# rsutormin/KmerGutsJava

Measured on AMD Instinct MI355X. Metric: amino-acid residues/sec scanned (and hits/sec) on 1 Gbp synthetic, 1/2/4/8 MI355X, higher is better.
Workload: dtype int64; 1 GPU; 1 Gbp contig mix (0.5 kbp..1.024 Mbp, uniform ACGT) on 1 GPU, 6-frame translate + 8-mer lookup vs 1400303159-slot signature table (33.6 GB, load 0.50), -m 5 -g 200; total_bp_rank0=1000000000, contigs_rank0=6351, total_bp_all_ranks=1000000000, num_sigs=1400303159, residues_rank0=1999974596, residues_all_ranks=1999974596, hits_rank0=36744843, hits_all_ranks=36744843, calls_rank0=4, parallelism=contig shards x1, table replicated

## Files before the change

kmergutsjava_amd/csrc/kg_host.hpp:

```cpp
#pragma once

#include <algorithm>
#include <atomic>
#include <cstdio>
#include <cstdlib>
#include <cstring>
#include <map>
#include <memory>
#include <mutex>
#include <new>
#include <optional>
#include <string>
#include <thread>
#include <unordered_map>
#include <vector>

namespace {

thread_local std::string g_err;

int fail(int code, const std::string &msg)
{
    g_err = msg;
    return code;
}

#define HIP_TRY(expr)                                                                              \
    do {                                                                                           \
        hipError_t e_ = (expr);                                                                    \
        if (e_ != hipSuccess)                                                                      \
            return fail(KG_ERR_DEVICE, std::string(#expr) + ": " + hipGetErrorString(e_));         \
    } while (0)

struct DevCache {
    std::mutex mu;
    std::multimap<size_t, void *> free_;
    std::unordered_map<void *, size_t> live;

    static size_t round_up(size_t b)
    {
        if (b < 256) return 256;
        size_t g = b >= (8u << 20) ? (2u << 20) : 256;
        return (b + g - 1) / g * g;
    }
    hipError_t get(void **p, size_t bytes)
    {
        bytes = round_up(bytes);
        std::lock_guard<std::mutex> lk(mu);
        auto it = free_.lower_bound(bytes);
        if (it != free_.end() && it->first <= bytes + bytes / 2 + (1u << 20)) {
            *p = it->second;
            live[*p] = it->first;
            free_.erase(it);
            return hipSuccess;
        }
        hipError_t e = hipMalloc(p, bytes);
        if (e != hipSuccess) {
            for (auto &kv : free_) (void)hipFree(kv.second);
            free_.clear();
            e = hipMalloc(p, bytes);
            if (e != hipSuccess) return e;
        }
        live[*p] = bytes;
        return hipSuccess;
    }
    void put(void *p)
    {
        std::lock_guard<std::mutex> lk(mu);
        auto it = live.find(p);
        if (it == live.end()) return;
        free_.emplace(it->second, p);
        live.erase(it);
    }
    void detach(void *p)
    {
        std::lock_guard<std::mutex> lk(mu);
        live.erase(p);
    }
    size_t live_bytes()
    {
        std::lock_guard<std::mutex> lk(mu);
        size_t n = 0;
        for (auto &kv : live) n += kv.second;
        return n;
    }
    void release_all()
    {
        std::lock_guard<std::mutex> lk(mu);
        for (auto &kv : free_) (void)hipFree(kv.second);
        for (auto &kv : live) (void)hipFree(kv.first);
        free_.clear();
        live.clear();
    }
    void release_free()
    {
        std::lock_guard<std::mutex> lk(mu);
        for (auto &kv : free_) (void)hipFree(kv.second);
        free_.clear();
    }
};

struct PinCache {
    std::mutex mu;
    std::multimap<size_t, void *> free_;
    std::unordered_map<void *, size_t> live;
    size_t kept = 0;
    static constexpr size_t kKeepTotal = 6ull << 30;

    hipError_t get(void **p, size_t bytes)
    {
        bytes = bytes < 4096 ? 4096 : (bytes + 4095) / 4096 * 4096;
        {
            std::lock_guard<std::mutex> lk(mu);
            auto it = free_.lower_bound(bytes);
            if (it != free_.end() && it->first <= 2 * bytes + (1u << 16)) {
                *p = it->second;
                live[*p] = it->first;
                kept -= it->first;
                free_.erase(it);
                return hipSuccess;
            }
        }
        hipError_t e = hipHostMalloc(p, bytes);
        if (e != hipSuccess) return e;
        std::lock_guard<std::mutex> lk(mu);
        live[*p] = bytes;
        return hipSuccess;
    }
    void put(void *p)
    {
        std::vector<void *> drop;
        {
            std::lock_guard<std::mutex> lk(mu);
            auto it = live.find(p);
            if (it == live.end()) return;
            const size_t bytes = it->second;
            live.erase(it);
            free_.emplace(bytes, p);
            kept += bytes;
            while (kept > kKeepTotal && !free_.empty()) {
                auto big = std::prev(free_.end());
                kept -= big->first;
                drop.push_back(big->second);
                free_.erase(big);
            }
        }
        for (void *d : drop) (void)hipHostFree(d);
    }
    void release_all()
    {
        std::lock_guard<std::mutex> lk(mu);
        for (auto &kv : free_) (void)hipHostFree(kv.second);
        for (auto &kv : live) (void)hipHostFree(kv.first);
        free_.clear();
        live.clear();
        kept = 0;
    }
};

}

constexpr uint64_t kHbitsMaxSlots = 1ull << 26;

constexpr uint32_t kMaxChunks = 8;
constexpr uint32_t kMaxOrderStreams = 4;
enum : int {
    kPevChunk = 0,
    kPevFork = 16,
    kPevJoin2 = 17, kPevJoin3 = 18,
    kPevTotals = 19,
    kPevVerified = 20,
    kPevBase = 32,
    kPevOrdered = 40,
    kPevCount = 48
};
static_assert(kPevChunk + 2 * kMaxChunks <= kPevFork && kPevVerified + kMaxChunks <= kPevBase && kPevBase + kMaxChunks <= kPevOrdered &&
              kPevOrdered + kMaxOrderStreams <= kPevCount, "event slots overlap");
enum : int { kEvBegin = 0, kEvScanBegin = 1, kEvScanEnd = 2, kEvOrderEnd = 3, kEvAggEnd = 4, kEvScattered = 5 , kEvSpare = 6,
             kEvJoined = 7 , kEvCount = 8, kEvStageBegin = kEvBegin, kEvStageEnd = kEvScanBegin };
enum : int { kTotHits = 0, kTotCursor = 1 , kTotValid = 2, kTotSlots = 3 ,
             kTotCalls = 4, kTotRanOff = 5 , kTotPieces = 6, kTotVoters = 7, kTotWords = 8,
             kTotSent = 6  };
enum : int { kPcUcur = 0 , kPcCcur = 8 , kPcBase = 16 ,
             kPcCtot = 32 , kPcWords = 48 };
static_assert(kPcUcur + kMaxChunks <= kPcCcur && kPcCcur + kMaxChunks <= kPcBase && kPcBase + kMaxChunks + 1 <= kPcCtot &&
              kPcCtot + kMaxChunks <= kPcWords, "per-chunk words overlap");
enum : int { kOvfGroups = 0 , kOvfLowc = 1 , kOvfGuard = 2 ,
             kOvfWords = 8 };
enum : int { kPinPc = 0 , kPinOvf = 48 , kPinTotals = 80 , kPinCalls = 88 ,
             kPinPieces = 89, kPinWords = 96,
             kPinStage = 80, kPinStageWords = kPinWords - kPinStage,
             kPinAssign = 90  };
static_assert(kPinPc + kPcWords <= kPinOvf && kOvfWords * kMaxChunks * 4 <= (kPinTotals - kPinOvf) * 8 && kPinTotals + kTotSent <= kPinCalls,
              "counters must fit their pinned words");
static_assert(kPinAssign >= kPinStage && kPinAssign + 2 + 3 <= kPinWords, "stage words must fit their pinned words");

struct kg_table {
    int device = 0;
    hipStream_t stream = nullptr;
    hipStream_t stream2 = nullptr;
    hipStream_t stream3 = nullptr;
    hipStream_t ostream[kMaxOrderStreams] = {};
    hipEvent_t pev[kPevCount] = {};
    bool own_entries = false;
    uint8_t *d_entries = nullptr;
    uint8_t *d_tags = nullptr;
    uint8_t *d_bidx = nullptr;
    bool bidx_exact = false;
    uint32_t *d_hbits = nullptr;
    uint64_t tail_start = 0;
    int64_t num_sigs = 0, entry_size = 0, version = 0;
    uint64_t limit = 0;
    uint64_t magic = 0;
    uint32_t m35 = 0;
    uint64_t occupied = 0;
    double stage_ratio = 1.0 / 16;
    size_t scatter_lds[2][3] = {};
    kg::ScatterCold *d_cold = nullptr;
    kg::ScatterCold h_cold[kMaxChunks] = {};
    kg::CallsCold *d_calls_cold = nullptr;
    kg::CallsCold h_calls_cold = {};
    size_t hist_lds = 48 * 1024;
    size_t place_lds[2] = {48 * 1024, 48 * 1024};
    hipEvent_t ev[kEvCount] = {};
    uint64_t *h_pin = nullptr;
    std::atomic<int> busy{0};
    uint32_t fail_alloc_at = 0, alloc_count = 0;
    DevCache cache;
    PinCache pins;
};

struct kg_result {
    kg_table *tab = nullptr;
    bool own_tab = false;
    kg_stats st = {};
    uint32_t per = 6;
    kg_hit *d_hits = nullptr;
    int64_t *d_chs = nullptr;
    kg_call *d_calls = nullptr;
    int64_t *d_ccs = nullptr;
    kg_otu *d_otu = nullptr;
    uint8_t *d_ev = nullptr, *d_tail_ev = nullptr;
    uint32_t *d_hit_slots = nullptr;
    bool has_progress = false;
    kg_progress progress = {};
    void *h_hits = nullptr, *h_chs = nullptr, *h_ccs = nullptr, *h_calls = nullptr, *h_otu = nullptr, *h_ev = nullptr,
         *h_tail_ev = nullptr, *h_hit_slots = nullptr;
};

namespace {

uint32_t env_u32(const char *name, uint32_t dflt)
{
    const char *v = getenv(name);
    if (!v || !*v) return dflt;
    char *end = nullptr;
    long x = strtol(v, &end, 10);
    return (end != v && x >= 0) ? (uint32_t)x : dflt;
}

constexpr uint32_t kMaxGrid = 256u * 32u;

uint32_t env_knob(const char *name, uint32_t dflt, uint32_t lo, uint32_t hi, uint32_t mult = 1)
{
    uint32_t x = dflt;
    if (const char *v = getenv(name); v && *v) {
        char *end = nullptr;
        const long long y = strtoll(v, &end, 10);
        if (end != v && y >= 0) x = y > (long long)hi ? hi : (uint32_t)y;
    }
    x = std::min(hi, std::max(lo, x));
    return (x + mult - 1) / mult * mult;
}

uint32_t test_hook(const char *name)
{
    static const bool enabled = env_u32("KG_ENABLE_TEST_HOOKS", 0u) != 0;
    return enabled ? env_u32(name, 0u) : 0u;
}

int dalloc(kg_table *t, void **p, size_t bytes)
{
    if (t->fail_alloc_at && ++t->alloc_count == t->fail_alloc_at)
        return fail(KG_ERR_NOMEM, "device allocation failed: KG_TEST_FAIL_ALLOC test hook");
    hipError_t e = t->cache.get(p, bytes);
    if (e != hipSuccess) return fail(KG_ERR_NOMEM, std::string("device allocation failed: ") + hipGetErrorString(e));
    return KG_OK;
}

void dfree(kg_table *t, void *p)
{
    if (p) t->cache.put(p);
}

int dalloc_detached(kg_table *t, uint8_t **p, size_t bytes)
{
    const int rc = dalloc(t, (void **)p, bytes);
    if (rc == KG_OK) t->cache.detach(*p);
    return rc;
}

struct Detached {
    uint8_t *p = nullptr;
    Detached() = default;
    Detached(const Detached &) = delete;
    Detached &operator=(const Detached &) = delete;
    ~Detached() { if (p) (void)hipFree(p); }
};

int table_new(int device, kg_table **out);

struct CallScope {
    kg_table *t = nullptr;
    const bool owned;
    int rc;
    CallScope(kg_table *tab, const char *busy_text) : owned(false), rc(tab->busy.exchange(1) != 0 ? fail(KG_ERR_BUSY, busy_text) : KG_OK)
    {
        if (rc == KG_OK) { t = tab; rc = arm(true); }
    }
    explicit CallScope(int device, bool hook = true) : owned(true), rc(table_new(device, &t))
    {
        if (rc == KG_OK) arm(hook);
    }
    ~CallScope()
    {
        if (!t) return;
        t->fail_alloc_at = 0;
        if (owned) kg_table_close(t);
        else t->busy.store(0);
    }
    int arm(bool hook)
    {
        t->fail_alloc_at = hook ? test_hook("KG_TEST_FAIL_ALLOC") : 0u;
        t->alloc_count = 0;
        if (!owned) HIP_TRY(hipSetDevice(t->device));
        return KG_OK;
    }
    kg_table *disown() { kg_table *out = t; t = nullptr; out->fail_alloc_at = 0; return out; }
};

int prefix_sum(kg_table *t, const uint32_t *d_in, uint64_t n, uint32_t *d_out, uint64_t *d_partial, uint64_t *d_total,
               hipStream_t stream = nullptr)
{
    if (!stream) stream = t->stream;
    uint32_t nb = (uint32_t)((n + kg::kScanChunk - 1) / kg::kScanChunk);
    if (nb == 0) nb = 1;
    hipLaunchKernelGGL(kg::scan_partials_kernel, dim3(nb), dim3(kg::kScanThreads), 0, stream, d_in, n, d_partial);
    hipLaunchKernelGGL(kg::scan_top_kernel, dim3(1), dim3(kg::kScanThreads), 0, stream, d_partial, nb, d_total);
    hipLaunchKernelGGL(kg::scan_final_kernel, dim3(nb), dim3(kg::kScanThreads), 0, stream, d_in, n, d_partial, d_out);
    HIP_TRY(hipGetLastError());
    return KG_OK;
}

struct ClearItem { void *p; uint64_t words; };

template <typename G>
int clear_words(hipStream_t stream, G grid, std::initializer_list<ClearItem> items)
{
    kg::ClearList cl = {};
    uint64_t most = 0;
    for (const ClearItem &it : items) {
        if (!it.words) continue;
        if (cl.n == (int)std::size(cl.p)) return fail(KG_ERR_DEVICE, "more than eight arrays in one clear (internal error)");
        cl.p[cl.n] = (uint32_t *)it.p; cl.words[cl.n++] = it.words;
        most = std::max(most, it.words);
    }
    if (cl.n) hipLaunchKernelGGL(kg::clear_many_kernel, dim3(grid(most)), dim3(256), 0, stream, cl);
    return KG_OK;
}

struct Scratch {
    kg_table *t;
    std::vector<void *> ptrs;
    explicit Scratch(kg_table *tt) : t(tt) {}
    ~Scratch()
    {
        (void)hipStreamSynchronize(t->stream);
        if (t->stream2) (void)hipStreamSynchronize(t->stream2);
        if (t->stream3) (void)hipStreamSynchronize(t->stream3);
        for (auto &os : t->ostream) if (os) (void)hipStreamSynchronize(os);
        for (void *p : ptrs) dfree(t, p);
    }
    void adopt(void *p) { ptrs.push_back(p); }
    void release(void *p) { ptrs.erase(std::find(ptrs.begin(), ptrs.end(), p)); }
    template <typename T> int get(T **p, size_t count)
    {
        void *v = nullptr;
        int rc = dalloc(t, &v, count * sizeof(T));
        if (rc) return rc;
        ptrs.push_back(v);
        *p = (T *)v;
        return KG_OK;
    }
};

struct SetBase {
    kg_table *tab = nullptr;
    bool own_tab = false;
    std::vector<void *> blocks;
    SetBase() = default;
    SetBase(const SetBase &) = delete;
    SetBase &operator=(const SetBase &) = delete;
    ~SetBase()
    {
        if (!tab) return;
        (void)hipSetDevice(tab->device);
        for (void *p : blocks) dfree(tab, p);
        if (own_tab) kg_table_close(tab);
    }
    template <typename T> T *keep(Scratch &sc, T *p)
    {
        if (p) { blocks.push_back(p); sc.release(p); }
        return p;
    }
};

template <typename S>
int make_set(const CallScope &cs, std::unique_ptr<S> &set)
{
    set.reset(new (std::nothrow) S());
    if (!set) return fail(KG_ERR_NOMEM, "out of host memory");
    set->tab = cs.t;
    return KG_OK;
}

template <typename S>
int hand_out(CallScope &cs, std::unique_ptr<S> &set, S **out)
{
    if (cs.owned) {
        cs.t->cache.release_free();
        set->own_tab = true;
        cs.disown();
    }
    *out = set.release();
    return KG_OK;
}

int device_of(const SetBase *s) { return s ? s->tab->device : 0; }

template <typename T>
int copy_records(const void *s, int device, const T *src, size_t per, int64_t have, int64_t first, int64_t count, T *dst, const char *what,
                 const char *of = "the set")
{
    if (!s || (count > 0 && !dst)) return fail(KG_ERR_ARG, "null argument");
    if (first < 0 || count < 0 || first + count > have) return fail(KG_ERR_ARG, std::string(what) + ": range outside " + of);
    if (count == 0) return KG_OK;
    HIP_TRY(hipSetDevice(device));
    HIP_TRY(hipMemcpy(dst, src + (size_t)first * per, (size_t)count * per * sizeof(T), hipMemcpyDefault));
    return KG_OK;
}

int copy_starts(const void *s, int device, const int64_t *src, int64_t n, int64_t *dst)
{
    if (!s || !dst) return fail(KG_ERR_ARG, "null argument");
    HIP_TRY(hipSetDevice(device));
    HIP_TRY(hipMemcpy(dst, src, ((size_t)n + 1) * 8, hipMemcpyDefault));
    return KG_OK;
}

template <typename St>
int copy_stats(const void *s, const St *st, St *out)
{
    if (!s || !out) return fail(KG_ERR_ARG, "null argument");
    *out = *st;
    return KG_OK;
}

uint32_t grid_of(uint64_t n, uint32_t threads = 256)
{
    return (uint32_t)std::max<uint64_t>(1, (n + threads - 1) / threads);
}

uint64_t magic_of(uint64_t d)
{
    return d == 1 ? ~0ull : (uint64_t)(((unsigned __int128)1 << 64) / d);
}

std::string kmer_text(int64_t v)
{
    char b[32];
    snprintf(b, sizeof b, "%lld", (long long)v);
    return b;
}

int fail_and_free(kg_result *r, int rc) { std::string keep = g_err; kg_result_free(r); g_err = keep; return rc; }

uint32_t bit_width(uint64_t v) { return v ? 64u - (uint32_t)__builtin_clzll(v) : 0u; }

uint32_t bits_for(uint64_t n) { return n > 1 ? bit_width(n - 1) : 0; }

template <int N>
struct Events {
    hipEvent_t e[N] = {};
    ~Events() { for (auto x : e) if (x) (void)hipEventDestroy(x); }
    int create() { for (auto &x : e) HIP_TRY(hipEventCreate(&x)); return KG_OK; }
    hipEvent_t operator[](int i) const { return e[i]; }
    float ms(int i, int j) const { float m = 0; (void)hipEventElapsedTime(&m, e[i], e[j]); return m; }
};

struct ErrWord { int word, code; const char *prefix, *suffix; };
constexpr uint64_t kNoErr = 0x7F7F7F7F7F7F7F7Full;
static_assert(kNoErr == kg::kAssignNoErr && kNoErr == kg::kRegionNoErr, "the stages' kernels share the error words' \"none\"");

int read_error_words(kg_table *t, const void *d_words, size_t n_words, int pin, std::initializer_list<ErrWord> table)
{
    HIP_TRY(hipMemcpyAsync(t->h_pin + pin, d_words, n_words * 8, hipMemcpyDeviceToHost, t->stream));
    HIP_TRY(hipStreamSynchronize(t->stream));
    for (const ErrWord &w : table)
        if (const uint64_t at = t->h_pin[pin + w.word]; at != kNoErr) return fail(w.code, w.prefix + kmer_text((int64_t)at) + w.suffix);
    return KG_OK;
}

int read_record_errors(kg_table *t, const void *d_words, size_t n_words, int n_err, const char *const *what)
{
    int rc;
    if ((rc = read_error_words(t, d_words, n_words, kPinStage, {}))) return rc;
    const uint64_t *h = t->h_pin + kPinStage;
    const int first = (int)(std::min_element(h, h + n_err) - h);
    if (h[first] != kNoErr) return fail(KG_ERR_ARG, "record " + kmer_text((int64_t)h[first]) + what[first]);
    return KG_OK;
}

int upload_pinned(kg_table *t, const uint8_t *src, size_t bytes, uint8_t *d_dst)
{
    const size_t CH = 32u << 20;
    const size_t n_pieces = (bytes + CH - 1) / CH;
    const unsigned hw = std::thread::hardware_concurrency();
    const size_t n_thr = std::max<size_t>(1, std::min<size_t>({(size_t)8, (size_t)(hw ? hw : 4), n_pieces}));
    std::atomic<size_t> next{0};
    std::atomic<bool> ok{true};
    auto worker = [&]() {
        if (hipSetDevice(t->device) != hipSuccess) { ok = false; return; }
        hipStream_t s = nullptr;
        uint8_t *pin[2] = {nullptr, nullptr};
        hipEvent_t done[2] = {nullptr, nullptr};
        bool good = hipStreamCreateWithFlags(&s, hipStreamNonBlocking) == hipSuccess &&
                    hipHostMalloc((void **)&pin[0], CH) == hipSuccess && hipHostMalloc((void **)&pin[1], CH) == hipSuccess &&
                    hipEventCreate(&done[0]) == hipSuccess && hipEventCreate(&done[1]) == hipSuccess;
        bool used[2] = {false, false};
        int which = 0;
        while (good && ok.load()) {
            const size_t k = next.fetch_add(1);
            if (k >= n_pieces) break;
            const size_t at = k * CH, n = std::min(CH, bytes - at);
            if (used[which]) good = hipEventSynchronize(done[which]) == hipSuccess;
            if (!good) break;
            memcpy(pin[which], src + at, n);
            good = hipMemcpyAsync(d_dst + at, pin[which], n, hipMemcpyHostToDevice, s) == hipSuccess &&
                   hipEventRecord(done[which], s) == hipSuccess;
            used[which] = true;
            which ^= 1;
        }
        if (s && hipStreamSynchronize(s) != hipSuccess) good = false;
        if (!good) ok = false;
        for (int i = 0; i < 2; i++) { if (pin[i]) (void)hipHostFree(pin[i]); if (done[i]) (void)hipEventDestroy(done[i]); }
        if (s) (void)hipStreamDestroy(s);
    };
    {
        std::vector<std::thread> pool;
        for (size_t i = 1; i < n_thr; i++) pool.emplace_back(worker);
        worker();
        for (auto &th : pool) th.join();
    }
    return ok.load() ? KG_OK : fail(KG_ERR_DEVICE, "uploading to the device failed (pinned staging or host-to-device copy)");
}

struct SortPairs {
    uint64_t *k[2] = {nullptr, nullptr};
    uint32_t *v[2] = {nullptr, nullptr};
    int cur = 0;
    int alloc(Scratch &sc, uint64_t n) { int rc = sc.get(&k[0], n); return rc ? rc : sc.get(&v[0], n); }
    uint64_t *keys() const { return k[cur]; }
    uint32_t *vals() const { return v[cur]; }
    SortPairs next() const { SortPairs s; s.k[0] = k[cur ^ 1]; s.v[0] = v[cur]; return s; }
    int sort(kg_table *t, Scratch &sc, uint64_t n, uint32_t key_bits);
};

int SortPairs::sort(kg_table *t, Scratch &sc, uint64_t n, uint32_t key_bits)
{
    if (n <= 1 || key_bits == 0) return KG_OK;
    const uint32_t n_tiles = (uint32_t)((n + kg::kBuildTile - 1) / kg::kBuildTile);
    const uint32_t passes = (key_bits + 7) / 8, bits = passes ? (key_bits + passes - 1) / passes : 1, radix = 1u << bits;
    const uint64_t n_hist = (uint64_t)radix * n_tiles;
    const uint64_t nb = (n_hist + kg::kScanChunk - 1) / kg::kScanChunk;
    uint32_t *hist = nullptr, *offs = nullptr;
    uint64_t *partial = nullptr;
    int rc;
    if ((rc = sc.get(&k[cur ^ 1], n)) || (rc = sc.get(&v[cur ^ 1], n)) || (rc = sc.get(&hist, n_hist)) ||
        (rc = sc.get(&offs, n_hist)) || (rc = sc.get(&partial, nb + 2)))
        return rc;
    for (uint32_t p = 0; p < passes; p++) {
        const uint32_t shift = p * bits;
        hipLaunchKernelGGL(kg::build_hist_kernel, dim3(n_tiles), dim3(kg::kBuildThreads), 0, t->stream, k[cur], n, shift, radix,
                           n_tiles, hist);
        HIP_TRY(hipGetLastError());
        if ((rc = prefix_sum(t, hist, n_hist, offs, partial, partial + nb + 1))) return rc;
        hipLaunchKernelGGL(kg::build_scatter_kernel, dim3(n_tiles), dim3(kg::kBuildThreads), 0, t->stream, k[cur], v[cur], n,
                           shift, bits, n_tiles, offs, k[cur ^ 1], v[cur ^ 1]);
        HIP_TRY(hipGetLastError());
        cur ^= 1;
    }
    return KG_OK;
}

}
```

kmergutsjava_amd/csrc/kg_host_plan.hpp:

```cpp
#pragma once

namespace {


template <typename T, T V, T... Vs, typename F>
void dispatch(T x, F &&f)
{
    if constexpr (sizeof...(Vs) == 0) f(std::integral_constant<T, V>{});
    else if (x == V) f(std::integral_constant<T, V>{});
    else dispatch<T, Vs...>(x, f);
}

struct BatchPlan {
    std::vector<uint32_t> ibase;
    uint64_t nblocks = 0, windows = 0, residues = 0;
    uint64_t n_rows = 0, n_cont = 0;
    int64_t longest = 0;
};

template <bool AA>
int plan_batch(const int64_t *offsets, int64_t n_seqs, BatchPlan &b)
{
    constexpr uint32_t PER = AA ? 1 : 6;
    b.ibase.resize((size_t)n_seqs + 1);
    for (int64_t k = 0; k < n_seqs; k++) {
        int64_t L = offsets[k + 1] - offsets[k];
        if (L < 0) return fail(KG_ERR_ARG, "offsets must be non-decreasing");
        b.longest = std::max(b.longest, L);
        if (L > 0xFFFFFFF0ll) return fail(KG_ERR_LIMIT, "a single sequence longer than 2^32-16 characters");
        b.ibase[(size_t)k] = (uint32_t)b.nblocks;
        uint64_t nb;
        if (AA) {
            uint64_t nwin = L >= 9 ? (uint64_t)L - 8 : 0;
            b.windows += nwin;
            b.residues += (uint64_t)L;
            nb = (nwin + kg::kAaWinPerBlock - 1) / kg::kAaWinPerBlock;
        } else {
            uint64_t npos = L >= 24 ? (uint64_t)L - 23 : 0;
            b.windows += 2 * npos;
            for (int f = 0; f < 3; f++)
                if (L - f >= 3) b.residues += 2 * (uint64_t)((L - f) / 3);
            nb = (npos + kg::kDnaPosPerBlock - 1) / kg::kDnaPosPerBlock;
        }
        b.nblocks += nb;
        if (b.nblocks > 0x7FFFFFFFull / PER) return fail(KG_ERR_LIMIT, "batch too large: more than 2^31-1 window rows; split the batch");
    }
    b.ibase[(size_t)n_seqs] = (uint32_t)b.nblocks;
    if (b.windows > 0xFFFFFF00ull) return fail(KG_ERR_LIMIT, "batch too large: more than 2^32-256 windows; split the batch");
    b.n_rows = b.nblocks * PER;
    b.n_cont = (uint64_t)n_seqs * PER;
    return KG_OK;
}

uint64_t bucket_count(uint64_t limit, uint32_t shift) { return (limit + (1ull << shift) - 1) >> shift; }

struct PartPlan {
    bool applicable = false;
    uint32_t shift = 0, buckets = 0;
    uint32_t n_chunks = 0;
    std::vector<uint64_t> clo;
    std::vector<int64_t> cseq;
    uint64_t max_chunk = 0;
    uint32_t n_wg = 0, cap = 0;
    uint64_t n_regions = 0;
    uint32_t ovf_cap = 0;
    uint32_t gshift = 10, groups_stride = 0;
    size_t next_stride = 0;
    size_t scatter_lds = 0;
    bool use_bidx = false, part_counters = false, prog_index = false;
    uint32_t probe_grid = 0, index_grid = 0, verify_grid = 0, lowc_grid = 0, ovf_grid = 0, order_grid = 0;
    uint32_t scatter_prio = 0, index_prio = 0, verify_prio = 0, index_r = 1, probe_grab = 0;
    uint32_t flush_list = 0;
    uint64_t list_slack = 0, ucap = 0, ccap = 0;
    uint32_t n_os = 0;
    bool early_totals = false, place_staged = false, debug = false;
};

template <bool AA>
int plan_partition(const kg_table *t, const BatchPlan &b, bool progress, bool counters_req, PartPlan &pl)
{
    constexpr uint32_t PER = AA ? 1 : 6;
    const uint64_t nblocks = b.nblocks;
    uint32_t shift = env_knob("KG_PART_SHIFT", 21u, 4u, 31u);
    const uint64_t qmax = (uint64_t)KG_MAX_ENCODED / (uint64_t)t->num_sigs + 1;
    while (shift > 4 && qmax >= (1ull << (32 - shift))) shift--;
    while (bucket_count(t->limit, shift) > (uint64_t)kg::kMaxBuckets) shift++;
    while (kg::scatter_lds_bytes<AA>((uint32_t)bucket_count(t->limit, shift)) > 160u * 1024) shift++;
    const bool fits = shift < 32 && qmax < (1ull << (32 - shift)) && nblocks <= (1ull << 23) && t->m35 != 0 &&
                      t->limit < (1ull << 32) - 64;
    const uint32_t mode = env_u32("KG_PARTITION", 2u);
    const bool worth = t->limit >= (64ull << 20) && b.windows >= (1ull << 27);
    if (!(fits && nblocks > 0 && (mode == 1 || (mode == 2 && worth)))) return KG_OK;
    pl.shift = shift;
    pl.buckets = (uint32_t)bucket_count(t->limit, shift);

    constexpr uint32_t WIN = AA ? 64u : 384u;
    uint32_t want = env_u32("KG_PART_CHUNKS", 4u);
    if (want < 1) want = 1;
    if (want > kMaxChunks) want = kMaxChunks;
    if (getenv("KG_PART_MIN_CHUNK_BLOCKS")) {
        const uint64_t min_chunk = std::max(1u, env_u32("KG_PART_MIN_CHUNK_BLOCKS", 600000u));
        while (want > 1 && nblocks / want < min_chunk) want--;
    } else {
        const uint32_t by_size = nblocks < 450000 ? 1u : std::max(2u, (uint32_t)std::lround(std::sqrt((double)nblocks / 325000.0)));
        want = std::min(want, std::max(1u, by_size));
    }
    pl.clo.push_back(0); pl.cseq.push_back(0);
    std::vector<double> cum;
    if (const char *tp = getenv("KG_PART_TAPER")) {
        double acc = 0;
        for (const char *q = tp; *q;) {
            char *endp = nullptr;
            const double v = strtod(q, &endp);
            if (endp == q) break;
            acc += v; cum.push_back(acc);
            q = *endp == ',' ? endp + 1 : endp;
        }
        if (cum.size() >= 2 && cum.size() <= kMaxChunks && acc > 0) { for (auto &x : cum) x /= acc; want = (uint32_t)cum.size(); }
        else cum.clear();
    }
    for (uint32_t c = 1; c < want; c++) {
        const uint64_t target = cum.empty() ? nblocks * c / want : (uint64_t)((double)nblocks * cum[c - 1]);
        const auto it = std::lower_bound(b.ibase.begin(), b.ibase.end(), (uint32_t)target);
        const uint64_t cut = *it;
        if (cut > pl.clo.back() && cut < nblocks) { pl.clo.push_back(cut); pl.cseq.push_back((int64_t)(it - b.ibase.begin())); }
    }
    pl.clo.push_back(nblocks); pl.cseq.push_back((int64_t)b.ibase.size() - 1);
    pl.n_chunks = (uint32_t)pl.clo.size() - 1;
    for (uint32_t c = 0; c < pl.n_chunks; c++) pl.max_chunk = std::max(pl.max_chunk, pl.clo[c + 1] - pl.clo[c]);
    const uint64_t max_chunk = pl.max_chunk;
    const uint64_t chunk_blocks = (max_chunk + kg::kScatterWaves - 1) / kg::kScatterWaves * kg::kScatterWaves;
    const double max_frac = (double)max_chunk / (double)nblocks;
    uint32_t n_wg = env_knob("KG_PART_WGS", 256u, 1u, kMaxGrid);
    if ((uint64_t)n_wg * kg::kScatterWaves > chunk_blocks) n_wg = (uint32_t)((chunk_blocks + kg::kScatterWaves - 1) / kg::kScatterWaves);
    const uint64_t blocks_per_wg = ((chunk_blocks + (uint64_t)n_wg * kg::kScatterWaves - 1) / ((uint64_t)n_wg * kg::kScatterWaves)) * kg::kScatterWaves;
    const double mean = (double)blocks_per_wg * WIN / (double)pl.buckets * (env_u32("KG_PART_SLACK", 100u) / 100.0);
    const uint64_t cap64 = ((uint64_t)(mean + 6.0 * std::sqrt(mean) + 32.0) + 15) / 16 * 16;
    if (cap64 >= (1ull << 24) || (uint64_t)pl.buckets * n_wg >= (1ull << 24)) return KG_OK;
    pl.n_wg = n_wg;
    pl.cap = (uint32_t)cap64;
    pl.n_regions = (uint64_t)pl.buckets * n_wg;
    pl.ovf_cap = env_u32("KG_PART_OVF_GROUPS", (uint32_t)std::min<uint64_t>(1u << 23, std::max<uint64_t>(65536, pl.n_regions * pl.cap / 16 / 8)));
    while (pl.gshift < 12 && ((max_chunk * PER) >> pl.gshift) + 2 > 8192) pl.gshift++;
    pl.groups_stride = (uint32_t)(((max_chunk * PER) >> pl.gshift) + 2);
    if (pl.groups_stride > kg::kMaxGroups) return fail(KG_ERR_LIMIT, "a chunk of the batch holds more than 2^26 window rows");
    pl.next_stride = std::max<size_t>((size_t)pl.buckets + 8, 256);
    pl.use_bidx = t->d_bidx != nullptr && !counters_req && env_u32("KG_BIDX", 1u) != 0;
    pl.part_counters = (counters_req || progress) && !pl.use_bidx;
    pl.prog_index = progress && pl.use_bidx;
    pl.scatter_lds = kg::scatter_lds_bytes<AA>(pl.buckets);
    pl.flush_list = env_knob("KG_SCATTER_FLUSH_LIST", kg::scatter_flush_list_max<AA>(), 1u, kg::scatter_flush_list_max<AA>());
    pl.probe_grid = env_knob("KG_PROBE_GRID", 256u * 8u, 8u, kMaxGrid, 8u);
    pl.index_grid = env_knob("KG_INDEX_GRID", 256u * 4u, 8u, kMaxGrid, 8u);
    pl.scatter_prio = std::min(3u, env_u32("KG_SCATTER_PRIO", 1u));
    pl.index_prio = std::min(3u, env_u32("KG_INDEX_PRIO", 2u));
    pl.verify_prio = std::min(3u, env_u32("KG_VERIFY_PRIO", pl.n_chunks == 1 ? 2u : 0u));
    uint32_t index_r = env_u32("KG_INDEX_R", 0u);
    if (index_r == 0) index_r = mean * 0.7 >= 640.0 ? 1u : mean * 0.7 >= 320.0 ? 2u : 4u;
    if (index_r != 1 && index_r != 2) index_r = 4;
    while (index_r > 1 && (n_wg % index_r != 0 || kg::kIndexN % index_r != 0)) index_r /= 2;
    pl.index_r = index_r;
    pl.verify_grid = env_knob("KG_VERIFY_GRID", 256u * 2u, 1u, kMaxGrid);
    pl.lowc_grid = env_knob("KG_LOWC_GRID", 256u, 1u, kMaxGrid);
    pl.ovf_grid = env_knob("KG_OVF_GRID", 256u, 1u, kMaxGrid);
    pl.list_slack = (uint64_t)(std::max(std::max(pl.probe_grid, pl.index_grid), pl.verify_grid) + 64) * 4 * kg::kUChunk + 4096;
    pl.ucap = ((uint64_t)((double)b.windows * t->stage_ratio * max_frac) + pl.list_slack + kg::kUChunk - 1) / kg::kUChunk * kg::kUChunk;
    pl.ccap = ((uint64_t)((double)b.windows * (t->stage_ratio * 1.25 + 0.03) * max_frac) + pl.list_slack + kg::kUChunk - 1) /
              kg::kUChunk * kg::kUChunk;
    if (test_hook("KG_TEST_TINY_LISTS")) pl.ucap = pl.ccap = kg::kUChunk;
    const uint32_t grab_unit = 256u * (uint32_t)std::max(kg::kProbeN, kg::kIndexN);
    pl.probe_grab = env_knob("KG_PROBE_GRAB", pl.cap, grab_unit, 1u << 24, grab_unit);
    pl.n_os = pl.n_chunks < 2 ? 0u : std::min(env_u32("KG_ORDER_STREAMS", 0u), kMaxOrderStreams);
    pl.early_totals = pl.n_os == 0 && env_u32("KG_EARLY_TOTALS", 1u) != 0;
    pl.order_grid = env_knob("KG_ORDER_GRID", 256u * 3u, 1u, kMaxGrid);
    pl.place_staged = pl.gshift == 10 && env_u32("KG_PLACE_STAGED", 1u) != 0;
    pl.debug = getenv("KG_DEBUG") != nullptr;
    pl.applicable = true;
    return KG_OK;
}

struct DirectPlan {
    uint32_t scan_grid, stage_chunk;
    const uint32_t *d_hbits;
    uint32_t rpg;
    uint64_t stage_cap;
};

template <bool AA>
DirectPlan plan_direct(const kg_table *t, const BatchPlan &b, bool counters)
{
    DirectPlan pl;
    pl.scan_grid = env_knob("KG_SCAN_GRID", 256u * 8u, 1u, kMaxGrid);
    pl.stage_chunk = env_knob("KG_STAGE_CHUNK", 256u, 1u, 1u << 12);
    const uint32_t filter_mode = env_u32("KG_DIRECT_FILTER", 1u);
    pl.d_hbits = (counters || filter_mode == 0 || (filter_mode == 1 && t->limit <= (4ull << 20))) ? nullptr : t->d_hbits;
    pl.rpg = AA ? 1u : env_u32("KG_SCAN_RPG", pl.d_hbits ? 6u : 3u);
    if (pl.rpg != 1 && pl.rpg != 2 && pl.rpg != 3 && pl.rpg != 6) pl.rpg = 3;
    pl.stage_cap = (uint64_t)((double)b.windows * t->stage_ratio) + 4096 + (uint64_t)pl.scan_grid * kg::kWavesPerWG * pl.stage_chunk;
    if (pl.stage_cap > 0xFFFFFF00ull) pl.stage_cap = 0xFFFFFF00ull;
    if (test_hook("KG_TEST_TINY_LISTS")) pl.stage_cap = 256;
    return pl;
}

struct AggPlan {
    uint32_t pshift;
    bool pieces_on;
    uint32_t agg_pairs;
};

AggPlan plan_aggregate()
{
    AggPlan pl;
    pl.pshift = std::min(20u, std::max(6u, env_u32("KG_AGG_BLOCK_SHIFT", 9u)));
    pl.pieces_on = env_u32("KG_AGG_PIECES", 1u) != 0;
    pl.agg_pairs = env_u32("KG_AGG_PAIRS", 1u);
    return pl;
}

}
```

kmergutsjava_amd/csrc/kg_host_scan.hpp:

```cpp
#pragma once

namespace {

struct ScanCtx {
    kg_table *t;
    kg_result *res;
    Scratch &sc;
    const BatchPlan &b;
    const uint8_t *d_seq, *h_seq;
    const int64_t *offsets;
    int64_t n_seqs;
    bool progress, counters;
    bool seq_uploaded;
    uint64_t n_hits = 0;
    int64_t *d_off = nullptr;
    uint32_t *d_ibase = nullptr;
    kg::BlockDesc *d_blocks = nullptr;
    uint32_t *d_counts = nullptr, *d_offs = nullptr, *d_bsb = nullptr;
    uint64_t *d_partial = nullptr, *d_totals = nullptr;
    kg::Progress *d_prog = nullptr;
};

int upload_seq(const ScanCtx &cx, int64_t a, int64_t b)
{
    if (cx.h_seq && b > a)
        HIP_TRY(hipMemcpyAsync(const_cast<uint8_t *>(cx.d_seq) + a, cx.h_seq + a, (size_t)(b - a), hipMemcpyHostToDevice, cx.t->stream));
    return KG_OK;
}

template <int N>
struct BlockGuard {
    Scratch &sc;
    void **slot[N];
    void release() { for (void **q : slot) { dfree(sc.t, *q); *q = nullptr; } }
    ~BlockGuard() { for (void **q : slot) if (*q) { sc.adopt(*q); *q = nullptr; } }
};

void drop_hits(kg_table *t, kg_result *res)
{
    dfree(t, res->d_hits); dfree(t, res->d_hit_slots);
    res->d_hits = nullptr; res->d_hit_slots = nullptr;
}

int send_counters(kg_table *t, const uint64_t *d_pc, const uint32_t *d_ovfc, const uint64_t *d_totals, hipStream_t s)
{
    if (d_pc) {
        HIP_TRY(hipMemcpyAsync(t->h_pin + kPinPc, d_pc, kPcWords * 8, hipMemcpyDeviceToHost, s));
        HIP_TRY(hipMemcpyAsync(t->h_pin + kPinOvf, d_ovfc, kOvfWords * kMaxChunks * 4, hipMemcpyDeviceToHost, s));
    }
    HIP_TRY(hipMemcpyAsync(t->h_pin + kPinTotals, d_totals, kTotSent * 8, hipMemcpyDeviceToHost, s));
    return KG_OK;
}

void note_totals(ScanCtx &cx, uint64_t n_hits, bool counted)
{
    kg_table *t = cx.t;
    kg_stats &st = cx.res->st;
    const uint64_t *h_tot = t->h_pin + kPinTotals;
    st.windows_valid = counted ? (int64_t)h_tot[kTotValid] : -1;
    st.slots_inspected = counted ? (int64_t)h_tot[kTotSlots] : -1;
    st.lookup_ran_off = h_tot[kTotRanOff] ? 1 : 0;
    if (cx.b.windows) {
        double ratio = (double)n_hits / (double)cx.b.windows * 1.1 + 1e-3;
        if (ratio > t->stage_ratio) t->stage_ratio = ratio > 1.0 ? 1.0 : ratio;
    }
    cx.n_hits = n_hits;
    st.n_hits = (int64_t)n_hits;
}

int progress_begin(ScanCtx &cx)
{
    kg_table *t = cx.t;
    int rc;
    if (t->limit > 0xFFFFFFFFull) return fail(KG_ERR_UNSUPPORTED, "KG_F_PROGRESS: table streams of 2^32 records or more");
    if ((rc = cx.sc.get(&cx.d_prog, 1))) return rc;
    kg::Progress h;
    for (auto &x : h.first) x = ~0ull;
    h.last_plus1 = 0; h.first_beyond = ~0ull; h.walk_ran_off = 0;
    for (auto &x : h.found_upto) x = 0;
    h.kmers_found = 0;
    for (auto &x : h.miss_max1) x = 0;
    const double n = (double)t->num_sigs;
    auto tenth = [&](uint64_t s) { return (int)(10.0 * ((double)(s + 1) / n)); };
    for (int f = 0; f <= 10; f++) {
        const unsigned __int128 num = (unsigned __int128)(uint64_t)t->num_sigs * (unsigned)f;
        uint64_t s = (uint64_t)((num + 9) / 10);
        s = s > 3 ? s - 3 : 0;
        while (tenth(s) < f) s++;
        h.lo[f] = s;
    }
    HIP_TRY(hipMemcpyAsync(cx.d_prog, &h, sizeof h, hipMemcpyHostToDevice, t->stream));
    HIP_TRY(hipStreamSynchronize(t->stream));
    return KG_OK;
}

int progress_finish(ScanCtx &cx, bool index_walks)
{
    kg_table *t = cx.t;
    int rc;
    if (index_walks)
        hipLaunchKernelGGL(kg::progress_finish_kernel, dim3(1), dim3(256), 0, t->stream, cx.d_prog, t->d_tags, t->limit);
    uint32_t *d_bitmap = nullptr;
    const uint64_t n_words = (t->limit + 31) / 32 + 1;
    if ((rc = cx.sc.get(&d_bitmap, (size_t)n_words))) return rc;
    HIP_TRY(hipMemsetAsync(d_bitmap, 0, n_words * 4, t->stream));
    if (cx.n_hits)
        hipLaunchKernelGGL(kg::mark_found_kernel, dim3((uint32_t)std::min<uint64_t>(2048, (cx.n_hits + 255) / 256)), dim3(256), 0, t->stream,
                           cx.res->d_hit_slots, cx.n_hits, d_bitmap);
    hipLaunchKernelGGL(kg::count_found_kernel, dim3((uint32_t)std::min<uint64_t>(2048, (n_words + 255) / 256)), dim3(256), 0, t->stream,
                       d_bitmap, n_words, cx.d_prog);
    return KG_OK;
}

int progress_fetch(ScanCtx &cx)
{
    kg::Progress h;
    HIP_TRY(hipMemcpy(&h, cx.d_prog, sizeof h, hipMemcpyDeviceToHost));
    kg_progress &g = cx.res->progress;
    for (int f = 0; f <= 10; f++) g.first_visited[f] = h.first[f] == ~0ull ? -1 : (int64_t)h.first[f];
    g.last_visited = (int64_t)h.last_plus1 - 1;
    g.first_beyond = h.first_beyond == ~0ull ? -1 : (int64_t)h.first_beyond;
    g.walk_ran_off = h.walk_ran_off ? 1 : 0;
    g.stream_slots = (int64_t)cx.t->limit;
    for (int f = 0; f <= 10; f++) g.found_upto[f] = g.first_visited[f] < 0 ? 0 : (int64_t)h.found_upto[f];
    g.kmers_found = (int64_t)h.kmers_found;
    cx.res->has_progress = true;
    return KG_OK;
}

struct PartBuffers {
    uint64_t *d_ent = nullptr, *d_ovf_ent = nullptr;
    uint32_t *d_fill = nullptr, *d_ovf_bucket = nullptr, *d_next = nullptr;
    uint32_t *d_ovfc = nullptr;
    uint32_t *d_lowc = nullptr;
    kg::RowGeo *d_geo = nullptr;
    uint64_t *d_pc = nullptr;
    uint32_t *d_ghist = nullptr, *d_gbase = nullptr, *d_gcur1 = nullptr, *d_gcur2 = nullptr, *d_gtile = nullptr;
    uint64_t ucap = 0, ccap = 0;
    size_t cused_stride = 0, candused_stride = 0;
    kg_hit *d_ulist = nullptr, *d_sortA = nullptr, *d_sortB = nullptr;
    uint32_t *d_cused = nullptr, *d_candused = nullptr;
    kg::CandRec *d_cand = nullptr;
};

struct ChunkView {
    uint32_t c, lo, nb;
    uint64_t *ent, *ovf_ent;
    uint32_t *fill, *next, *ovfc, *ovf_bucket;
    kg_hit *ulist, *sortA, *sortB;
    uint32_t *cused, *candused;
    kg::CandRec *cand;
    unsigned long long *ucur, *ccur;
    uint64_t *base, *ctot;
    uint32_t *ghist, *gbase, *gcur1, *gcur2, *gtile;
};

ChunkView chunk_view(const PartPlan &pl, const PartBuffers &pb, uint32_t c)
{
    ChunkView v;
    v.c = c; v.lo = (uint32_t)pl.clo[c]; v.nb = (uint32_t)(pl.clo[c + 1] - pl.clo[c]);
    v.ent = pb.d_ent + (uint64_t)c * pl.n_regions * pl.cap;
    v.fill = pb.d_fill + (uint64_t)c * pl.n_regions;
    v.next = pb.d_next + (size_t)c * pl.next_stride;
    v.ovfc = pb.d_ovfc + kOvfWords * c; v.ovf_bucket = pb.d_ovf_bucket + (size_t)c * pl.ovf_cap;
    v.ovf_ent = pb.d_ovf_ent + (size_t)c * pl.ovf_cap * kg::kGroup;
    v.ulist = pb.d_ulist + (uint64_t)c * pb.ucap;
    v.cused = pb.d_cused + c * pb.cused_stride; v.candused = pb.d_candused + c * pb.candused_stride;
    v.cand = pb.d_cand + (uint64_t)c * pb.ccap;
    v.ucur = (unsigned long long *)(pb.d_pc + kPcUcur + c); v.ccur = (unsigned long long *)(pb.d_pc + kPcCcur + c);
    v.base = pb.d_pc + kPcBase + c; v.ctot = pb.d_pc + kPcCtot + c;
    v.ghist = pb.d_ghist + (size_t)c * pl.groups_stride; v.gbase = pb.d_gbase + (size_t)c * (pl.groups_stride + 1);
    v.gcur1 = pb.d_gcur1 + (size_t)c * (kg::kHDigits + 1); v.gcur2 = pb.d_gcur2 + (size_t)c * pl.groups_stride;
    v.gtile = pb.d_gtile + (size_t)c * (kg::kHDigits + 1);
    v.sortA = pb.d_sortA + (uint64_t)c * pb.ucap; v.sortB = pb.d_sortB + (uint64_t)c * pb.ucap;
    return v;
}

int scatter_variant_of(const ScanCtx &cx)
{
    return cx.t->limit >= (uint64_t)cx.t->num_sigs ? 0 : cx.d_prog ? 2 : 1;
}
template <typename F>
void scatter_variant(int variant, F &&f)
{
    if (variant == 0) f(std::false_type{}, std::false_type{});
    else if (variant == 1) f(std::true_type{}, std::false_type{});
    else f(std::true_type{}, std::true_type{});
}

int upload_scatter_cold(const ScanCtx &cx, const PartPlan &pl, const PartBuffers &pb)
{
    kg_table *t = cx.t;
    kg::ScatterCold h[kMaxChunks] = {};
    for (uint32_t c = 0; c < pl.n_chunks; c++) {
        uint32_t *ovfc = pb.d_ovfc + kOvfWords * c;
        h[c].ovf_cursor = ovfc; h[c].ovf_bucket = pb.d_ovf_bucket + (size_t)c * pl.ovf_cap;
        h[c].ovf_ent = pb.d_ovf_ent + (size_t)c * pl.ovf_cap * kg::kGroup;
        h[c].lowc_cursor = ovfc + kOvfLowc; h[c].lowc_blocks = pb.d_lowc + pl.clo[c];
        h[c].ctr = (unsigned long long *)(cx.d_totals + kTotValid); h[c].prog = cx.d_prog;
        h[c].ovf_cap = pl.ovf_cap;
    }
    if (!t->d_cold) HIP_TRY(hipMalloc((void **)&t->d_cold, sizeof h));
    else if (!memcmp(h, t->h_cold, sizeof h)) return KG_OK;
    memcpy(t->h_cold, h, sizeof h);
    HIP_TRY(hipMemcpyAsync(t->d_cold, t->h_cold, sizeof h, hipMemcpyHostToDevice, t->stream));
    return KG_OK;
}

template <bool AA>
int chunk_passes(const ScanCtx &cx, const PartPlan &pl, const PartBuffers &pb, const ChunkView &v)
{
    kg_table *t = cx.t;
    kg::Progress *d_prog = cx.d_prog;
    unsigned long long *d_ctr = (unsigned long long *)(cx.d_totals + kTotValid);
    const hipStream_t s2 = t->stream2, s3 = t->stream3;
    uint32_t *lowc_cursor = v.ovfc + kOvfLowc, *lowc = pb.d_lowc + v.lo;
    const uint32_t limit32 = (uint32_t)std::min<uint64_t>(t->limit, 0xFFFFFFFFull);
    scatter_variant(scatter_variant_of(cx), [&](auto is_short, auto prog) {
        constexpr bool SHORT = decltype(is_short)::value, PROG = decltype(prog)::value;
        hipLaunchKernelGGL((kg::part_scatter_kernel<AA, SHORT, PROG>), dim3(pl.n_wg), dim3(kg::kWave * kg::kScatterWaves), pl.scatter_lds,
                           t->stream, cx.d_seq, cx.d_blocks, v.lo, v.nb, limit32, (uint32_t)t->num_sigs, t->m35, pl.shift, pl.buckets, pl.cap,
                           v.ent, v.fill, t->d_cold + v.c, pl.scatter_prio, pl.flush_list);
    });
    HIP_TRY(hipEventRecord(t->pev[kPevChunk + 2 * v.c], t->stream));
    HIP_TRY(hipStreamWaitEvent(s2, t->pev[kPevChunk + 2 * v.c], 0));
    hipLaunchKernelGGL((kg::lowc_blocks_kernel<AA>), dim3(pl.lowc_grid), dim3(64 * kg::kLowcWaves), 0, s2, cx.d_seq, cx.d_blocks, lowc_cursor, lowc,
                       t->limit, (uint32_t)t->num_sigs, t->m35, pl.shift, pl.n_wg, pl.cap, v.ent, v.fill, v.ovfc, pl.ovf_cap,
                       v.ovf_bucket, v.ovf_ent, d_ctr, d_prog);
    if (pl.use_bidx) {
        const uint32_t tail_start = (uint32_t)std::min<uint64_t>(t->tail_start, 0xFFFFFFFFull);
        dispatch<int, 1, 2, 4>((int)pl.index_r, [&](auto r) {
            dispatch<bool, true, false>(t->bidx_exact, [&](auto exact) {
                dispatch<bool, true, false>(pl.prog_index, [&](auto prog) {
                    constexpr int R = decltype(r)::value;
                    constexpr bool EXACT = decltype(exact)::value, PROG = decltype(prog)::value;
                    hipLaunchKernelGGL((kg::bucket_index_kernel<kg::kIndexN, R, EXACT, PROG>), dim3(pl.index_grid), dim3(256), 0, s2,
                                       t->d_bidx, tail_start, v.ent, v.fill, pl.n_wg, pl.cap, pl.buckets, pl.shift, pl.probe_grab, v.next,
                                       v.cand, v.candused, v.ccur, pb.ccap, d_ctr, pl.index_prio, PROG ? d_prog : (kg::Progress *)nullptr);
                });
            });
        });
    } else {
        dispatch<bool, true, false>(pl.part_counters, [&](auto counters) {
            constexpr bool COUNTERS = decltype(counters)::value;
            hipLaunchKernelGGL((kg::bucket_tag_kernel<COUNTERS>), dim3(pl.probe_grid), dim3(256), 0, s2, t->d_tags, t->limit,
                               (uint64_t)t->num_sigs, v.ent, v.fill, pl.n_wg, pl.cap, pl.buckets, pl.shift, pl.probe_grab, v.next, v.cand,
                               v.candused, v.ccur, pb.ccap, d_ctr, COUNTERS ? d_prog : (kg::Progress *)nullptr);
        });
    }
    HIP_TRY(hipEventRecord(t->pev[kPevChunk + 2 * v.c + 1], s2));
    HIP_TRY(hipStreamWaitEvent(s3, t->pev[kPevChunk + 2 * v.c + 1], 0));
    dispatch<int, 1, 2, 0>(pl.part_counters ? 1 : pl.prog_index ? 2 : 0, [&](auto walks) {
        constexpr bool COUNTERS = decltype(walks)::value == 1, PROG = decltype(walks)::value == 2;
        hipLaunchKernelGGL((kg::verify_kernel<AA, COUNTERS, PROG>), dim3(pl.verify_grid), dim3(256), 0, s3, t->d_entries, t->d_tags, t->limit,
                           (uint64_t)t->num_sigs, t->magic, v.cand, v.candused, v.ccur, pb.ccap, v.ulist, v.cused, v.ucur, pb.ucap, d_ctr,
                           d_prog, pl.verify_prio);
        hipLaunchKernelGGL((kg::overflow_probe_kernel<AA, COUNTERS, PROG>), dim3(pl.ovf_grid), dim3(256), 0, s3, t->d_entries, t->d_tags,
                           t->limit, (uint64_t)t->num_sigs, t->magic, v.ovf_bucket, v.ovf_ent, v.ovfc, pl.ovf_cap, pl.shift, v.ulist,
                           v.cused, v.ucur, pb.ucap, d_ctr, d_prog);
    });
    HIP_TRY(hipEventRecord(t->pev[kPevVerified + v.c], s3));
    HIP_TRY(hipGetLastError());
    return KG_OK;
}

template <bool AA>
int chunk_order(const ScanCtx &cx, const PartPlan &pl, const PartBuffers &pb, const ChunkView &v, uint64_t hits_cap)
{
    constexpr uint32_t PER = AA ? 1 : 6;
    kg_table *t = cx.t;
    kg_result *res = cx.res;
    const uint32_t c = v.c, gshift = pl.gshift;
    const bool last = c + 1 == pl.n_chunks;
    hipStream_t s = t->stream;
    if (pl.n_os) {
        s = t->ostream[c % pl.n_os];
        HIP_TRY(hipStreamWaitEvent(s, t->ev[kEvScattered], 0));
    }
    HIP_TRY(hipStreamWaitEvent(s, t->pev[kPevVerified + c], 0));
    const uint64_t row_lo = (uint64_t)v.lo * PER, row_hi = row_lo + (uint64_t)v.nb * PER;
    const uint32_t g0 = (uint32_t)(row_lo >> gshift);
    const uint32_t n_groups = v.nb ? (uint32_t)(((row_hi - 1) >> gshift) - g0 + 1) : 1u;
    hipLaunchKernelGGL(kg::hit_hist_kernel, dim3(pl.order_grid), dim3(kg::kHThreads), (size_t)n_groups * 4, s, v.ulist, v.cused, v.ucur, pb.ucap,
                       g0, 6u + gshift, n_groups, v.ghist);
    hipLaunchKernelGGL(kg::group_scan_kernel, dim3(1), dim3(kg::kGsThreads), 0, s, v.ghist, n_groups, v.gbase, v.gcur1, v.gcur2, v.ctot, v.gtile);
    if (pl.n_os && c) HIP_TRY(hipStreamWaitEvent(s, t->pev[kPevBase + c - 1], 0));
    hipLaunchKernelGGL(kg::chunk_base_kernel, dim3(1), dim3(1), 0, s, v.ctot, v.base, last ? cx.d_totals : (uint64_t *)nullptr);
    if (pl.n_os) HIP_TRY(hipEventRecord(t->pev[kPevBase + c], s));
    if (pl.early_totals && last) {
        int rc;
        if ((rc = send_counters(t, pb.d_pc, pb.d_ovfc, cx.d_totals, s))) return rc;
        HIP_TRY(hipEventRecord(t->pev[kPevTotals], s));
    }
    hipLaunchKernelGGL((kg::hit_partition_kernel<true>), dim3(pl.order_grid), dim3(kg::kHThreads), 0, s, v.ulist, v.cused, v.ucur, pb.ucap,
                       v.gbase, n_groups, g0, 6u + gshift, v.gcur1, v.sortA, pb.ucap, v.gtile);
    hipLaunchKernelGGL((kg::hit_partition_kernel<false>), dim3(pl.order_grid), dim3(kg::kHThreads), 0, s, v.sortA, v.cused, v.ucur, pb.ucap,
                       v.gbase, n_groups, g0, 6u + gshift, v.gcur2, v.sortB, pb.ucap, v.gtile);
    hipLaunchKernelGGL((kg::group_place_kernel<AA>), dim3(std::min(n_groups, 256u * 8u)), dim3(kg::kHThreads),
                       kg::group_place_lds(gshift, pl.place_staged), s,
                       v.sortB, v.gbase, n_groups, g0, gshift, (uint32_t)row_lo, (uint32_t)row_hi, pb.d_geo, (uint64_t)cx.b.n_rows,
                       pl.place_staged ? 1u : 0u, v.base, res->d_hits, hits_cap, cx.d_offs, res->d_hit_slots);
    HIP_TRY(hipGetLastError());
    return KG_OK;
}

template <bool AA>
int part_allocate(ScanCtx &cx, const PartPlan &pl, PartBuffers &pb)
{
    kg_table *t = cx.t;
    Scratch &sc = cx.sc;
    const uint32_t n_chunks = pl.n_chunks, groups_stride = pl.groups_stride;
    int rc;
    if ((rc = sc.get(&pb.d_ent, (size_t)(pl.n_regions * pl.cap * n_chunks)))) return rc;
    if ((rc = sc.get(&pb.d_fill, (size_t)pl.n_regions * n_chunks))) return rc;
    if ((rc = sc.get(&pb.d_ovf_ent, (size_t)pl.ovf_cap * kg::kGroup * n_chunks))) return rc;
    if ((rc = sc.get(&pb.d_ovf_bucket, (size_t)pl.ovf_cap * n_chunks))) return rc;
    if ((rc = sc.get(&pb.d_next, pl.next_stride * n_chunks))) return rc;
    if ((rc = sc.get(&pb.d_ovfc, kOvfWords * kMaxChunks))) return rc;
    if ((rc = sc.get(&pb.d_lowc, (size_t)cx.b.nblocks + 1))) return rc;
    if ((rc = sc.get(&pb.d_geo, (size_t)cx.b.n_rows))) return rc;
    if ((rc = sc.get(&pb.d_ghist, (size_t)groups_stride * n_chunks))) return rc;
    if ((rc = sc.get(&pb.d_gbase, (size_t)(groups_stride + 1) * n_chunks))) return rc;
    if ((rc = sc.get(&pb.d_gcur1, (size_t)(kg::kHDigits + 1) * n_chunks))) return rc;
    if ((rc = sc.get(&pb.d_gcur2, (size_t)groups_stride * n_chunks))) return rc;
    if ((rc = sc.get(&pb.d_gtile, (size_t)(kg::kHDigits + 1) * n_chunks))) return rc;
    if (kg::group_place_lds(pl.gshift, pl.gshift == 10) > t->place_lds[AA ? 1 : 0]) {
        const size_t want_lds = kg::group_place_lds(pl.gshift, pl.gshift == 10);
        HIP_TRY(hipFuncSetAttribute((const void *)kg::group_place_kernel<AA>, hipFuncAttributeMaxDynamicSharedMemorySize, (int)want_lds));
        t->place_lds[AA ? 1 : 0] = want_lds;
    }
    if (groups_stride * 4u > t->hist_lds) {
        HIP_TRY(hipFuncSetAttribute((const void *)kg::hit_hist_kernel, hipFuncAttributeMaxDynamicSharedMemorySize, (int)(groups_stride * 4u)));
        t->hist_lds = groups_stride * 4u;
    }
    if ((rc = sc.get(&pb.d_pc, kPcWords))) return rc;
    const int sv = scatter_variant_of(cx);
    if (t->scatter_lds[AA ? 1 : 0][sv] < pl.scatter_lds) {
        hipError_t e = hipSuccess;
        scatter_variant(sv, [&](auto is_short, auto prog) {
            e = hipFuncSetAttribute((const void *)kg::part_scatter_kernel<AA, decltype(is_short)::value, decltype(prog)::value>,
                                    hipFuncAttributeMaxDynamicSharedMemorySize, (int)pl.scatter_lds);
        });
        HIP_TRY(e);
        t->scatter_lds[AA ? 1 : 0][sv] = pl.scatter_lds;
    }
    return KG_OK;
}

template <bool AA>
int scan_partitioned(ScanCtx &cx, const PartPlan &pl, bool &done)
{
    constexpr uint32_t PER = AA ? 1 : 6;
    kg_table *t = cx.t;
    kg_result *res = cx.res;
    kg_stats &st = res->st;
    const uint32_t n_chunks = pl.n_chunks;
    const uint64_t nblocks = cx.b.nblocks;
    int rc;
    PartBuffers pb;
    if ((rc = part_allocate<AA>(cx, pl, pb))) return rc;
    BlockGuard<6> lists{cx.sc, {(void **)&pb.d_ulist, (void **)&pb.d_cused, (void **)&pb.d_cand, (void **)&pb.d_candused,
                                (void **)&pb.d_sortA, (void **)&pb.d_sortB}};
    pb.ucap = pl.ucap; pb.ccap = pl.ccap;
    HIP_TRY(hipEventRecord(t->ev[kEvScanBegin], t->stream));
    for (int attempt = 0; attempt < 3; attempt++) {
        const uint64_t ucap = pb.ucap, ccap = pb.ccap;
        const uint64_t hits_cap = ucap * n_chunks;
        pb.cused_stride = (size_t)(ucap / kg::kUChunk + 1); pb.candused_stride = (size_t)(ccap / kg::kUChunk + 1);
        if ((rc = dalloc(t, (void **)&res->d_hits, hits_cap * sizeof(kg_hit)))) return rc;
        if (cx.progress && (rc = dalloc(t, (void **)&res->d_hit_slots, hits_cap * 4))) return rc;
        if ((rc = dalloc(t, (void **)&pb.d_ulist, ucap * n_chunks * sizeof(kg_hit)))) return rc;
        if ((rc = dalloc(t, (void **)&pb.d_cused, pb.cused_stride * n_chunks * 4))) return rc;
        if ((rc = dalloc(t, (void **)&pb.d_cand, ccap * n_chunks * sizeof(kg::CandRec)))) return rc;
        if ((rc = dalloc(t, (void **)&pb.d_candused, pb.candused_stride * n_chunks * 4))) return rc;
        if ((rc = dalloc(t, (void **)&pb.d_sortA, ucap * n_chunks * sizeof(kg_hit)))) return rc;
        if ((rc = dalloc(t, (void **)&pb.d_sortB, ucap * n_chunks * sizeof(kg_hit)))) return rc;
        if ((rc = clear_words(t->stream, [](uint64_t most) { return (uint32_t)std::min<uint64_t>(4096, (most / 4 + 255) / 256 + 1); },
                              {{pb.d_cused, (uint64_t)pb.cused_stride * n_chunks},
                               {pb.d_candused, (uint64_t)pb.candused_stride * n_chunks},
                               {pb.d_pc, kPcWords * 2},
                               {cx.d_totals, kTotWords * 2},
                               {pb.d_ovfc, kOvfWords * kMaxChunks},
                               {pb.d_next, (uint64_t)pl.next_stride * n_chunks},
                               {pb.d_ghist, (uint64_t)pl.groups_stride * n_chunks}})))
            return rc;
        if ((rc = upload_scatter_cold(cx, pl, pb))) return rc;
        HIP_TRY(hipEventRecord(t->pev[kPevFork], t->stream));
        HIP_TRY(hipStreamWaitEvent(t->stream2, t->pev[kPevFork], 0));
        HIP_TRY(hipStreamWaitEvent(t->stream3, t->pev[kPevFork], 0));
        hipLaunchKernelGGL((kg::row_geo_kernel<AA>), dim3((uint32_t)((nblocks * PER + 255) / 256)), dim3(256), 0, t->stream3, cx.d_blocks,
                           (uint32_t)nblocks, pb.d_geo);
        for (uint32_t c = 0; c < n_chunks; c++) {
            if (!cx.seq_uploaded && (rc = upload_seq(cx, cx.offsets[pl.cseq[c]], cx.offsets[pl.cseq[c + 1]]))) return rc;
            if ((rc = chunk_passes<AA>(cx, pl, pb, chunk_view(pl, pb, c)))) return rc;
        }
        HIP_TRY(hipEventRecord(t->ev[kEvScattered], t->stream));
        cx.seq_uploaded = true;
        for (uint32_t k = 0; k < pl.n_os; k++)
            if (!t->ostream[k]) {
                int pr_least = 0, pr_greatest = 0;
                HIP_TRY(hipDeviceGetStreamPriorityRange(&pr_least, &pr_greatest));
                HIP_TRY(hipStreamCreateWithPriority(&t->ostream[k], hipStreamNonBlocking, pr_least));
            }
        for (uint32_t c = 0; c < n_chunks; c++)
            if ((rc = chunk_order<AA>(cx, pl, pb, chunk_view(pl, pb, c), hits_cap))) return rc;

        for (uint32_t k = 0; k < pl.n_os; k++) {
            HIP_TRY(hipEventRecord(t->pev[kPevOrdered + k], t->ostream[k]));
            HIP_TRY(hipStreamWaitEvent(t->stream, t->pev[kPevOrdered + k], 0));
        }
        HIP_TRY(hipEventRecord(t->pev[kPevJoin2], t->stream2));
        HIP_TRY(hipStreamWaitEvent(t->stream, t->pev[kPevJoin2], 0));
        HIP_TRY(hipEventRecord(t->pev[kPevJoin3], t->stream3));
        HIP_TRY(hipStreamWaitEvent(t->stream, t->pev[kPevJoin3], 0));
        HIP_TRY(hipEventRecord(t->ev[kEvJoined], t->stream));
        st.scan_launches++;
        HIP_TRY(hipEventRecord(t->ev[kEvScanEnd], t->stream));
        if (pl.early_totals) {
            HIP_TRY(hipEventSynchronize(t->pev[kPevTotals]));
        } else {
            if ((rc = send_counters(t, pb.d_pc, pb.d_ovfc, cx.d_totals, t->stream))) return rc;
            HIP_TRY(hipStreamSynchronize(t->stream));
        }
        const uint64_t *h_pc = t->h_pin + kPinPc;
        const uint32_t *h_ovf = reinterpret_cast<const uint32_t *>(t->h_pin + kPinOvf);
        uint64_t need_u = 0, need_c = 0;
        uint32_t max_ovf = 0, guard = 0;
        for (uint32_t c = 0; c < n_chunks; c++) {
            need_u = std::max(need_u, h_pc[kPcUcur + c]); need_c = std::max(need_c, h_pc[kPcCcur + c]);
            max_ovf = std::max(max_ovf, h_ovf[kOvfWords * c + kOvfGroups]);
            guard |= h_ovf[kOvfWords * c + kOvfGuard];
        }
        const uint64_t n_hits = h_pc[kPcBase + n_chunks];
        if (pl.debug)
            fprintf(stderr, "[kg] partition attempt %d: %u chunks (largest %llu of %llu blocks), overflow groups <= %u (cap %u), hit list <= %llu "
                            "(cap %llu), candidates <= %llu (cap %llu), regions/chunk %llu x %u entries, %u buckets, shift %u, %u scatter "
                            "workgroups, hits %llu, %s\n",
                    attempt, n_chunks, (unsigned long long)pl.max_chunk, (unsigned long long)nblocks, max_ovf, pl.ovf_cap,
                    (unsigned long long)need_u, (unsigned long long)ucap, (unsigned long long)need_c, (unsigned long long)ccap,
                    (unsigned long long)pl.n_regions, pl.cap, pl.buckets, pl.shift, pl.n_wg, (unsigned long long)n_hits, pl.use_bidx ? "byte home index" : "tags");
        const bool redo = guard || max_ovf > pl.ovf_cap || need_u > ucap || need_c > ccap;
        if (redo && pl.early_totals) HIP_TRY(hipStreamSynchronize(t->stream));
        if (guard || max_ovf > pl.ovf_cap) {
            st.fallback = guard ? 2 : 1;
            lists.release();
            drop_hits(t, res);
            return KG_OK;
        }
        if (!redo) {
            note_totals(cx, n_hits, pl.part_counters);
            st.partitioned = 1;
            st.part_chunks = (int32_t)n_chunks; st.part_buckets = (int32_t)pl.buckets; st.part_shift = (int32_t)pl.shift;
            st.part_levels = pl.use_bidx ? 4 : 1;
            done = true;
            return KG_OK;
        }
        lists.release();
        drop_hits(t, res);
        if (attempt == 2) break;
        if (need_c > ccap) { pb.ccap = (need_c + pl.list_slack + kg::kUChunk - 1) / kg::kUChunk * kg::kUChunk; pb.ucap = std::max(ucap, pb.ccap); }
        else pb.ucap = (need_u + pl.list_slack + kg::kUChunk - 1) / kg::kUChunk * kg::kUChunk;
    }
    return fail(KG_ERR_DEVICE, "hit list overflow after resize (internal error)");
}

template <bool AA>
int scan_direct(ScanCtx &cx, const DirectPlan &pl)
{
    kg_table *t = cx.t;
    kg_result *res = cx.res;
    kg_stats &st = res->st;
    const uint64_t nblocks = cx.b.nblocks, n_rows = cx.b.n_rows;
    int rc;
    st.scan_launches = 0;
    if (!cx.seq_uploaded) { if ((rc = upload_seq(cx, cx.offsets[0], cx.offsets[cx.n_seqs]))) return rc; cx.seq_uploaded = true; }
    uint64_t stage_cap = pl.stage_cap;
    kg_hit *d_stage = nullptr;
    uint32_t *d_stage_slot = nullptr;
    BlockGuard<2> stage{cx.sc, {(void **)&d_stage, (void **)&d_stage_slot}};
    unsigned long long *d_cursor = (unsigned long long *)(cx.d_totals + kTotCursor);
    unsigned long long *d_ctr = (unsigned long long *)(cx.d_totals + kTotValid);
    for (int attempt = 0;; attempt++) {
        if ((rc = dalloc(t, (void **)&d_stage, stage_cap * sizeof(kg_hit)))) return rc;
        if (cx.progress && (rc = dalloc(t, (void **)&d_stage_slot, stage_cap * 4))) return rc;
        HIP_TRY(hipMemsetAsync(cx.d_totals, 0, kTotWords * 8, t->stream));
        HIP_TRY(hipEventRecord(t->ev[kEvScanBegin], t->stream));
        if (nblocks) {
            const uint64_t wgs = (nblocks + kg::kWavesPerWG - 1) / kg::kWavesPerWG;
            const uint32_t grid = (uint32_t)(wgs < pl.scan_grid ? wgs : pl.scan_grid);
            dispatch<bool, true, false>(cx.counters, [&](auto counters) {
                dispatch<int, 1, 2, 3, 6>((int)pl.rpg, [&](auto rpg) {
                    constexpr bool COUNTERS = decltype(counters)::value;
                    constexpr int RPG = AA ? 1 : decltype(rpg)::value;
                    hipLaunchKernelGGL((kg::scan_kernel<AA, COUNTERS, RPG>), dim3(grid), dim3(kg::kWave * kg::kWavesPerWG), 0, t->stream,
                                       t->d_entries, t->d_tags, t->limit, (uint64_t)t->num_sigs, t->magic, t->m35, cx.d_seq, cx.d_blocks,
                                       (uint32_t)nblocks, cx.d_counts, cx.d_bsb, d_stage, d_cursor, stage_cap, pl.stage_chunk, d_ctr, cx.d_prog,
                                       d_stage_slot, pl.d_hbits, t->tail_start);
                });
            });
            HIP_TRY(hipGetLastError());
        }
        HIP_TRY(hipEventRecord(t->ev[kEvScanEnd], t->stream));
        st.scan_launches++;
        if ((rc = prefix_sum(t, cx.d_counts, n_rows, cx.d_offs, cx.d_partial, cx.d_totals + kTotHits))) return rc;
        if ((rc = send_counters(t, nullptr, nullptr, cx.d_totals, t->stream))) return rc;
        HIP_TRY(hipStreamSynchronize(t->stream));
        const uint64_t need = t->h_pin[kPinTotals + kTotCursor];
        if (need <= stage_cap) break;
        stage.release();
        if (attempt == 1) return fail(KG_ERR_DEVICE, "staging overflow after resize (internal error)");
        stage_cap = need;
    }
    const uint64_t n_hits = n_rows ? t->h_pin[kPinTotals + kTotHits] : 0;
    note_totals(cx, n_hits, cx.counters);

    if ((rc = dalloc(t, (void **)&res->d_hits, n_hits * sizeof(kg_hit)))) return rc;
    if (cx.progress && (rc = dalloc(t, (void **)&res->d_hit_slots, (n_hits ? n_hits : 1) * 4))) return rc;
    if (nblocks) {
        const uint32_t grid = (uint32_t)((nblocks + kg::kWavesPerWG - 1) / kg::kWavesPerWG);
        hipLaunchKernelGGL((kg::place_kernel<AA>), dim3(grid), dim3(kg::kWave * kg::kWavesPerWG), 0, t->stream, cx.d_blocks,
                           (uint32_t)nblocks, cx.d_counts, cx.d_offs, cx.d_bsb, pl.rpg, d_stage, res->d_hits, d_stage_slot, res->d_hit_slots);
    }
    return KG_OK;
}

template <bool AA>
int scan_impl(kg_table *t, const kg_params *p, const uint8_t *d_seq, const uint8_t *h_seq ,
              const int64_t *offsets, int64_t n_seqs, kg_result *res)
{
    constexpr uint32_t PER = AA ? 1 : 6;
    const bool progress = (p->flags & KG_F_PROGRESS) != 0;
    const bool counters_req = (p->flags & KG_F_COUNTERS) != 0;
    const bool aggregate = !(p->flags & KG_F_SKIP_AGGREGATE);
    kg_stats &st = res->st;
    res->per = PER;
    int rc;

    BatchPlan b;
    if ((rc = plan_batch<AA>(offsets, n_seqs, b))) return rc;
    const uint64_t nblocks = b.nblocks, n_rows = b.n_rows, n_cont = b.n_cont;
    st.n_seqs = n_seqs; st.n_containers = (int64_t)n_cont; st.n_blocks = (int64_t)nblocks;
    st.residues = (int64_t)b.residues; st.windows = (int64_t)b.windows;
    st.table_bytes = t->num_sigs * (int64_t)KG_TABLE_ENTRY_SIZE;

    Scratch sc(t);
    ScanCtx cx{t, res, sc, b, d_seq, h_seq, offsets, n_seqs, progress, counters_req || progress, h_seq == nullptr};
    if ((rc = sc.get(&cx.d_off, (size_t)n_seqs + 1))) return rc;
    if ((rc = sc.get(&cx.d_ibase, (size_t)n_seqs + 1))) return rc;
    HIP_TRY(hipMemcpyAsync(cx.d_off, offsets, ((size_t)n_seqs + 1) * 8, hipMemcpyHostToDevice, t->stream));
    HIP_TRY(hipMemcpyAsync(cx.d_ibase, b.ibase.data(), ((size_t)n_seqs + 1) * 4, hipMemcpyHostToDevice, t->stream));
    if ((rc = sc.get(&cx.d_blocks, nblocks))) return rc;
    if ((rc = sc.get(&cx.d_counts, n_rows))) return rc;
    if ((rc = sc.get(&cx.d_offs, n_rows))) return rc;
    if ((rc = sc.get(&cx.d_bsb, nblocks * 6))) return rc;
    if ((rc = sc.get(&cx.d_partial, (size_t)(std::max(n_rows, n_cont) / kg::kScanChunk + 2)))) return rc;
    if ((rc = sc.get(&cx.d_totals, kTotWords))) return rc;
    HIP_TRY(hipMemsetAsync(cx.d_totals, 0, kTotWords * 8, t->stream));
    if ((rc = dalloc(t, (void **)&res->d_chs, (n_cont + 1) * 8))) return rc;
    if (progress && (rc = progress_begin(cx))) return rc;
    HIP_TRY(hipEventRecord(t->ev[kEvBegin], t->stream));
    if (nblocks) {
        hipLaunchKernelGGL(kg::build_blocks_kernel, dim3((uint32_t)((nblocks + 255) / 256)), dim3(256), 0, t->stream,
                           cx.d_off, cx.d_ibase, (uint32_t)n_seqs, (uint32_t)nblocks, cx.d_blocks);
        HIP_TRY(hipGetLastError());
    }

    st.scan_launches = 0;
    PartPlan part;
    if ((rc = plan_partition<AA>(t, b, progress, counters_req, part))) return rc;
    bool part_done = false;
    if (part.applicable && (rc = scan_partitioned<AA>(cx, part, part_done))) return rc;
    if (!part_done && (rc = scan_direct<AA>(cx, plan_direct<AA>(t, b, cx.counters)))) return rc;

    if (progress && (rc = progress_finish(cx, part_done && part.prog_index))) return rc;
    hipLaunchKernelGGL((kg::container_starts_kernel<AA>), dim3((uint32_t)((n_cont + 1 + 255) / 256)), dim3(256), 0, t->stream,
                       cx.d_ibase, (uint32_t)n_seqs, cx.d_offs, n_rows, cx.d_totals, res->d_chs);
    HIP_TRY(hipGetLastError());
    HIP_TRY(hipEventRecord(t->ev[kEvOrderEnd], t->stream));

    if (aggregate && (rc = aggregate_stage(t, p, res, sc, n_seqs, n_cont, cx.n_hits, PER, cx.d_partial, cx.d_totals, nullptr, b.longest < (1ll << 30),
                                         plan_aggregate())))
        return rc;
    HIP_TRY(hipEventRecord(t->ev[kEvAggEnd], t->stream));
    HIP_TRY(hipStreamSynchronize(t->stream));
    st.n_calls = aggregate ? (int64_t)t->h_pin[kPinCalls] : 0;
    if (progress && (rc = progress_fetch(cx))) return rc;
    st.agg_pieces = aggregate ? (int32_t)std::min<uint64_t>(t->h_pin[kPinPieces], 0x7FFFFFFF) : 0;
    float ms = 0;
    HIP_TRY(hipEventElapsedTime(&ms, t->ev[kEvScanBegin], t->ev[kEvScanEnd])); st.ms_scan = ms;
    HIP_TRY(hipEventElapsedTime(&ms, t->ev[kEvScanEnd], t->ev[kEvOrderEnd])); st.ms_order = ms;
    HIP_TRY(hipEventElapsedTime(&ms, t->ev[kEvOrderEnd], t->ev[kEvAggEnd])); st.ms_aggregate = ms;
    HIP_TRY(hipEventElapsedTime(&ms, t->ev[kEvBegin], t->ev[kEvAggEnd])); st.ms_total = ms;
    if (st.partitioned) {
        HIP_TRY(hipEventElapsedTime(&ms, t->ev[kEvScanBegin], t->ev[kEvScattered])); st.ms_part_scatter = ms;
        st.ms_part_tag = 0;
        HIP_TRY(hipEventElapsedTime(&ms, t->ev[kEvScattered], t->ev[kEvJoined])); st.ms_part_verify = ms;
    }
    return KG_OK;
}

int scan_entry(kg_table *t, const kg_params *p, const uint8_t *seq, bool on_device, const int64_t *offsets, int64_t n_seqs,
               kg_result **out)
{
    if (!t || !p || !offsets || !out || n_seqs < 0) return fail(KG_ERR_ARG, "null or negative argument");
    if (n_seqs > 0x7FFFFFF0ll / 6) return fail(KG_ERR_LIMIT, "too many sequences in one batch");
    if (p->min_hits < 2)
        return fail(KG_ERR_UNSUPPORTED, "minHits < 2: the reference throws in processSetOfHits (KGJ:442); refusing");
    CallScope cs(t, "another kg_scan* is in flight on this kg_table (one scan at a time per table; open a second table "
                    "object for concurrent scans)");
    if (cs.rc) return cs.rc;
    int64_t total = offsets[n_seqs] - offsets[0];
    if (total < 0) return fail(KG_ERR_ARG, "offsets must be non-decreasing");
    if (!seq && total > 0) return fail(KG_ERR_ARG, "null sequence buffer");
    kg_result *r = new (std::nothrow) kg_result();
    if (!r) return fail(KG_ERR_NOMEM, "out of host memory");
    r->tab = t;
    uint8_t *d_seq = nullptr;
    int rc = KG_OK;
    if (!on_device) {
        size_t end = (size_t)offsets[n_seqs];
        rc = dalloc(t, (void **)&d_seq, end + 16);
    }
    if (rc == KG_OK) {
        const uint8_t *s = on_device ? seq : d_seq;
        const uint8_t *h = on_device ? nullptr : seq;
        rc = p->aa ? scan_impl<true>(t, p, s, h, offsets, n_seqs, r) : scan_impl<false>(t, p, s, h, offsets, n_seqs, r);
    }
    (void)hipStreamSynchronize(t->stream);
    if (d_seq) dfree(t, d_seq);
    if (rc != KG_OK) return fail_and_free(r, rc);
    *out = r;
    return KG_OK;
}

}

extern "C" {

int kg_scan(kg_table *t, const kg_params *p, const uint8_t *seq, const int64_t *offsets, int64_t n_seqs, kg_result **out)
{
    return scan_entry(t, p, seq, false, offsets, n_seqs, out);
}

int kg_scan_device(kg_table *t, const kg_params *p, const uint8_t *d_seq, const int64_t *offsets, int64_t n_seqs,
                   kg_result **out)
{
    return scan_entry(t, p, d_seq, true, offsets, n_seqs, out);
}

}
```

kmergutsjava_amd/csrc/kg_order.hpp:

```cpp
#pragma once

#include "kg_device.hpp"
#include "kg_partition.hpp"

namespace kg {

constexpr uint32_t kHThreads = 512;
constexpr uint32_t kHPer = 4;
constexpr uint32_t kHTile = kHThreads * kHPer;
constexpr uint32_t kHDigits = 128;
constexpr uint32_t kMaxGroups = kHDigits * kHDigits;

struct RowGeo { uint32_t container; int32_t pos_first; };

template <bool AA>
__global__ void row_geo_kernel(const BlockDesc *__restrict__ blocks, uint32_t n_blocks, RowGeo *__restrict__ geo)
{
    constexpr uint32_t ROWS = AA ? 1 : 6;
    const uint64_t tl = (uint64_t)blockIdx.x * blockDim.x + threadIdx.x;
    if (tl >= (uint64_t)n_blocks * ROWS) return;
    const uint32_t r = (uint32_t)(tl / n_blocks), it = (uint32_t)(tl % n_blocks);
    const BlockDesc bd = blocks[it];
    RowGeo g;
    int32_t pos0;
    row_record_key<AA>(bd, (int)r, 0, &g.container, &pos0);
    g.pos_first = (!AA && r >= 3) ? pos0 - 63 : pos0;
    geo[row_index<AA>(bd, it, (int)r)] = g;
}

__global__ __launch_bounds__(kHThreads) void hit_hist_kernel(const kg_hit *__restrict__ ulist, const uint32_t *__restrict__ chunk_used,
                                                             const unsigned long long *__restrict__ cursor, uint64_t ulist_cap,
                                                             uint32_t g0, uint32_t gs , uint32_t n_groups,
                                                             uint32_t *ghist )
{
    extern __shared__ uint32_t h_lds[];
    for (uint32_t g = threadIdx.x; g < n_groups; g += kHThreads) h_lds[g] = 0;
    __syncthreads();
    const unsigned long long cur = *cursor;
    const uint32_t n_chunks = (uint32_t)((cur < ulist_cap ? cur : ulist_cap) / kUChunk);
    for (uint32_t c = blockIdx.x; c < n_chunks; c += gridDim.x) {
        const uint32_t used = chunk_used[c];
        for (uint32_t k = threadIdx.x; k < used; k += kHThreads) {
            const uint32_t g = (ulist[(uint64_t)c * kUChunk + k].container >> gs) - g0;
            if (g < n_groups) atomicAdd(&h_lds[g], 1u);
        }
    }
    __syncthreads();
    for (uint32_t g = threadIdx.x; g < n_groups; g += kHThreads)
        if (h_lds[g]) atomicAdd(&ghist[g], h_lds[g]);
}

constexpr uint32_t kGsThreads = 256, kGsPer = 4;
__global__ __launch_bounds__(kGsThreads) void group_scan_kernel(const uint32_t *__restrict__ ghist, uint32_t n_groups, uint32_t *__restrict__ gbase,
                                                                uint32_t *__restrict__ cur1, uint32_t *__restrict__ cur2, uint64_t *total_out,
                                                                uint32_t *__restrict__ tile_start)
{
    __shared__ uint32_t wsum[kGsThreads / 64];
    __shared__ uint32_t carry;
    if (threadIdx.x == 0) carry = 0;
    __syncthreads();
    const int lane = threadIdx.x & 63, wave = threadIdx.x >> 6;
    for (uint32_t b = 0; b < n_groups; b += kGsThreads * kGsPer) {
        const uint32_t i0 = b + threadIdx.x * kGsPer;
        uint32_t x[kGsPer], mine = 0;
#pragma unroll
        for (uint32_t k = 0; k < kGsPer; k++) {
            x[k] = i0 + k < n_groups ? ghist[i0 + k] : 0u;
            mine += x[k];
        }
        uint32_t incl = mine;
        for (int off = 1; off < 64; off <<= 1) {
            const uint32_t y = __shfl_up(incl, off);
            if (lane >= off) incl += y;
        }
        if (lane == 63) wsum[wave] = incl;
        __syncthreads();
        uint32_t wbase = 0, all = 0;
        for (int w = 0; w < (int)(kGsThreads / 64); w++) {
            const uint32_t sw = wsum[w];
            if (w < wave) wbase += sw;
            all += sw;
        }
        const uint32_t c = carry;
        uint32_t e = c + wbase + incl - mine;
#pragma unroll
        for (uint32_t k = 0; k < kGsPer; k++) {
            const uint32_t i = i0 + k;
            if (i < n_groups) {
                gbase[i] = e;
                cur2[i] = e;
                if ((i & (kHDigits - 1)) == 0) cur1[i / kHDigits] = e;
            }
            e += x[k];
        }
        __syncthreads();
        if (threadIdx.x == 0) carry = c + all;
        __syncthreads();
    }
    const uint32_t n_d1 = (n_groups + kHDigits - 1) / kHDigits;
    if (threadIdx.x == 0) {
        gbase[n_groups] = carry;
        cur1[n_d1] = carry;
        *total_out = carry;
    }
    __syncthreads();
    const uint32_t d = threadIdx.x;
    const uint32_t t = d < n_d1 ? (cur1[d + 1] - cur1[d] + kHTile - 1) / kHTile : 0u;
    uint32_t incl = t;
    for (int off = 1; off < 64; off <<= 1) {
        const uint32_t y = __shfl_up(incl, off);
        if (lane >= off) incl += y;
    }
    if (d == 63) wsum[0] = incl;
    __syncthreads();
    if (d < kHDigits) {
        const uint32_t before = d >= 64 ? wsum[0] : 0u;
        tile_start[d] = before + incl - t;
        if (d == kHDigits - 1) tile_start[kHDigits] = before + incl;
    }
}

template <bool FIRST>
__global__ __launch_bounds__(kHThreads) void hit_partition_kernel(const kg_hit *__restrict__ in, const uint32_t *__restrict__ chunk_used,
                                                                  const unsigned long long *__restrict__ cursor, uint64_t in_cap,
                                                                  const uint32_t *__restrict__ gbase, uint32_t n_groups, uint32_t g0, uint32_t gs,
                                                                  uint32_t *cur, kg_hit *__restrict__ out, uint64_t out_cap,
                                                                  const uint32_t *__restrict__ tile_start)
{
    __shared__ __attribute__((aligned(16))) kg_hit stage[kHTile];
    __shared__ uint32_t hist[kHDigits], cnt[kHDigits], sbase[kHDigits], gb[kHDigits];
    const uint32_t tid = threadIdx.x, lane = tid & 63u, wave = tid >> 6;
    if (tid < kHDigits) hist[tid] = 0;
    const uint32_t n_d1 = (n_groups + kHDigits - 1) / kHDigits;
    uint32_t n_res = 0;
    if (FIRST) {
        const unsigned long long cc = *cursor;
        n_res = (uint32_t)((cc < in_cap ? cc : in_cap) / kUChunk);
    }
    __shared__ uint32_t tstart[kHDigits + 1];
    if (!FIRST) {
        if (tid <= kHDigits) tstart[tid] = tile_start[tid];
        __syncthreads();
    }
    const uint32_t n_items = FIRST ? (n_res + kHTile / kUChunk - 1) / (kHTile / kUChunk) : tstart[kHDigits];
    {
        for (uint32_t item = blockIdx.x; item < n_items; item += gridDim.x) {
            uint32_t d1 = 0, tile = item;
            if (!FIRST) {
                uint32_t lo_d = 0, hi_d = n_d1;
                while (hi_d - lo_d > 1) {
                    const uint32_t mid = (lo_d + hi_d) / 2;
                    if (tstart[mid] <= item) lo_d = mid; else hi_d = mid;
                }
                d1 = lo_d;
                tile = item - tstart[d1];
            }
            const uint32_t seg_lo = FIRST ? 0u : gbase[d1 * kHDigits];
            const uint32_t seg_hi = FIRST ? 0u : gbase[min((d1 + 1) * kHDigits, n_groups)];
            kg_hit rec[kHPer];
            uint32_t dr[kHPer];
#pragma unroll
            for (uint32_t k = 0; k < kHPer; k++) {
                const uint32_t i = k * kHThreads + tid;
                bool ok;
                uint64_t at;
                if (FIRST) {
                    const uint32_t c = tile * (kHTile / kUChunk) + i / kUChunk;
                    ok = c < n_res && (i % kUChunk) < chunk_used[c];
                    at = (uint64_t)c * kUChunk + (i % kUChunk);
                } else {
                    at = (uint64_t)seg_lo + (uint64_t)tile * kHTile + i;
                    ok = at < seg_hi;
                }
                dr[k] = ~0u;
                if (ok) {
                    rec[k] = stream_load_hit(in + at);
                    const uint32_t g = (rec[k].container >> gs) - g0;
                    if (g < n_groups) {
                        const uint32_t d = FIRST ? g / kHDigits : g % kHDigits;
                        dr[k] = (d << 16) | atomicAdd(&hist[d], 1u);
                    }
                }
            }
            __syncthreads();
            if (tid < kHDigits) {
                const uint32_t c = hist[tid];
                uint32_t incl = c;
                for (int off = 1; off < 64; off <<= 1) {
                    const uint32_t y = __shfl_up(incl, off);
                    if ((int)lane >= off) incl += y;
                }
                cnt[tid] = c;
                sbase[tid] = incl - c;
                gb[tid] = c ? atomicAdd(&cur[FIRST ? tid : d1 * kHDigits + tid], c) : 0u;
                hist[tid] = 0;
            }
            __syncthreads();
            const uint32_t first_half = sbase[63] + cnt[63];
#pragma unroll
            for (uint32_t k = 0; k < kHPer; k++)
                if (dr[k] != ~0u) {
                    const uint32_t d = dr[k] >> 16;
                    stage[sbase[d] + (d >= 64 ? first_half : 0u) + (dr[k] & 0xFFFFu)] = rec[k];
                }
            __syncthreads();
            const uint64_t *stage64 = reinterpret_cast<const uint64_t *>(stage);
            uint64_t *out64 = reinterpret_cast<uint64_t *>(out);
            for (uint32_t d = wave; d < kHDigits; d += kHThreads / 64u) {
                const uint32_t n = cnt[d];
                if (n == 0) continue;
                const uint32_t s0 = sbase[d] + (d >= 64 ? first_half : 0u);
                const uint64_t o0 = gb[d];
                const uint32_t n_ok = o0 >= out_cap ? 0u : (uint32_t)min((uint64_t)n, out_cap - o0);
                for (uint32_t i = lane; i < 3u * n_ok; i += 64u) stream_store8(out64 + o0 * 3u + i, stage64[(uint64_t)s0 * 3u + i]);
            }
            __syncthreads();
        }
    }
}

constexpr uint32_t kPlaceOut = 1536;
__host__ __device__ inline size_t group_place_lds(uint32_t gshift, bool staged)
{
    return staged ? ((size_t)20 << gshift) + (size_t)kPlaceOut * sizeof(kg_hit) : ((size_t)12 << gshift);
}
template <bool AA>
__global__ __launch_bounds__(kHThreads) void group_place_kernel(const kg_hit *__restrict__ in, const uint32_t *__restrict__ gbase, uint32_t n_groups,
                                                                uint32_t g0, uint32_t gshift, uint32_t row_lo, uint32_t row_hi ,
                                                                const RowGeo *__restrict__ geo, uint64_t n_rows_all, uint32_t staged,
                                                                const uint64_t *__restrict__ base,
                                                                kg_hit *__restrict__ hits, uint64_t hits_cap, uint32_t *__restrict__ offs,
                                                                uint32_t *__restrict__ hit_slots )
{
    extern __shared__ __attribute__((aligned(16))) unsigned char p_lds[];
    const uint32_t R = 1u << gshift;
    unsigned long long *masks = reinterpret_cast<unsigned long long *>(p_lds);
    uint32_t *pre = reinterpret_cast<uint32_t *>(masks + R);
    RowGeo *lgeo = reinterpret_cast<RowGeo *>(pre + R);
    uint64_t *lout = reinterpret_cast<uint64_t *>(lgeo + R);
    __shared__ uint32_t wsum[kHThreads / 64];
    const uint32_t tid = threadIdx.x, lane = tid & 63u, wave = tid >> 6;
    const uint64_t chunk_base = *base;
    const uint32_t per = R / kHThreads > 0 ? R / kHThreads : 1u;
    for (uint32_t g = blockIdx.x; g < n_groups; g += gridDim.x) {
        const uint32_t lo = gbase[g], n = gbase[g + 1] - lo;
        const uint64_t row0 = (uint64_t)(g0 + g) << gshift;
        const bool to_lds = staged && n <= kPlaceOut;
        for (uint32_t i = tid; i < R; i += kHThreads) {
            masks[i] = 0ull;
            if (staged && n && row0 + i < n_rows_all) lgeo[i] = geo[row0 + i];
        }
        __syncthreads();
        constexpr uint32_t kKeep = 4;
        const bool keep = n <= kHThreads * kKeep;
        kg_hit rk[kKeep];
        if (keep) {
#pragma unroll
            for (uint32_t j = 0; j < kKeep; j++) {
                const uint32_t k = j * kHThreads + tid;
                if (k < n) {
                    rk[j] = stream_load_hit(in + lo + k);
                    atomicOr(&masks[(rk[j].container >> 6) & (R - 1u)], 1ull << (rk[j].container & 63u));
                }
            }
        } else {
            for (uint32_t k = tid; k < n; k += kHThreads) {
                const uint32_t key = in[lo + k].container;
                atomicOr(&masks[(key >> 6) & (R - 1u)], 1ull << (key & 63u));
            }
        }
        __syncthreads();
        uint32_t mine = 0;
        const uint32_t r_lo = tid * per;
        if (r_lo < R)
            for (uint32_t i = 0; i < per; i++) mine += (uint32_t)__popcll(masks[r_lo + i]);
        uint32_t incl = mine;
        for (int off = 1; off < 64; off <<= 1) {
            const uint32_t y = __shfl_up(incl, off);
            if ((int)lane >= off) incl += y;
        }
        if (lane == 63) wsum[wave] = incl;
        __syncthreads();
        uint32_t run = incl - mine;
        for (uint32_t w = 0; w < wave; w++) run += wsum[w];
        if (r_lo < R)
            for (uint32_t i = 0; i < per; i++) {
                pre[r_lo + i] = run;
                const uint64_t row = row0 + r_lo + i;
                if (row >= row_lo && row < row_hi) offs[row] = (uint32_t)(chunk_base + lo + run);
                run += (uint32_t)__popcll(masks[r_lo + i]);
            }
        __syncthreads();
        auto place = [&](kg_hit h) {
            const uint32_t key = h.container, rl = (key >> 6) & (R - 1u), ol = key & 63u;
            const RowGeo gr = staged ? lgeo[rl] : geo[key >> 6];
            const uint32_t rank = pre[rl] + (uint32_t)__popcll(masks[rl] & ((1ull << ol) - 1ull));
            if (hit_slots && chunk_base + lo + rank < hits_cap)
                hit_slots[chunk_base + lo + rank] = (uint32_t)h.from0InProt;
            h.container = gr.container;
            h.from0InProt = gr.pos_first + (int32_t)ol;
            if (to_lds) {
                uint64_t w3[3];
                __builtin_memcpy(w3, &h, 24);
                lout[3u * rank] = w3[0]; lout[3u * rank + 1] = w3[1]; lout[3u * rank + 2] = w3[2];
            } else {
                const uint64_t dst = chunk_base + lo + rank;
                if (dst < hits_cap) hits[dst] = h;
            }
        };
        if (keep) {
#pragma unroll
            for (uint32_t j = 0; j < kKeep; j++)
                if (j * kHThreads + tid < n) place(rk[j]);
        } else {
            for (uint32_t k = tid; k < n; k += kHThreads) place(in[lo + k]);
        }
        __syncthreads();
        if (to_lds) {
            const uint64_t dst0 = chunk_base + lo;
            const uint32_t n_ok = dst0 >= hits_cap ? 0u : (uint32_t)min((uint64_t)n, hits_cap - dst0);
            uint64_t *out64 = reinterpret_cast<uint64_t *>(hits) + dst0 * 3u;
            for (uint32_t i = tid; i < 3u * n_ok; i += kHThreads) stream_store8(out64 + i, lout[i]);
            __syncthreads();
        }
    }
}

__global__ __launch_bounds__(256) void restore_hits_kernel(const kg_hit *__restrict__ src, uint64_t n_hits, const int64_t *__restrict__ seq_first,
                                                           uint64_t n_seqs, const int64_t *__restrict__ dst_first,
                                                           const int32_t *__restrict__ container_shift, kg_hit *__restrict__ dst)
{
    __shared__ uint64_t k_first;
    constexpr uint64_t kTile = 1024;
    const uint64_t n_tiles = (n_hits + kTile - 1) / kTile;
    for (uint64_t tile = blockIdx.x; tile < n_tiles; tile += gridDim.x) {
        __syncthreads();
        if (threadIdx.x == 0) {
            const uint64_t i0 = tile * kTile;
            uint64_t lo = 0, hi = n_seqs;
            while (hi - lo > 1) {
                const uint64_t mid = lo + (hi - lo) / 2;
                if ((uint64_t)seq_first[mid] <= i0) lo = mid; else hi = mid;
            }
            k_first = lo;
        }
        __syncthreads();
        uint64_t k = k_first;
#pragma unroll
        for (int j = 0; j < 4; j++) {
            const uint64_t i = tile * kTile + (uint64_t)j * 256 + threadIdx.x;
            if (i < n_hits) {
                while (k + 1 < n_seqs && (uint64_t)seq_first[k + 1] <= i) k++;
                kg_hit h = src[i];
                h.container += (uint32_t)container_shift[k];
                dst[(uint64_t)dst_first[k] + (i - (uint64_t)seq_first[k])] = h;
            }
        }
    }
}

}
```

kmergutsjava_amd/csrc/kg_partition.hpp:

```cpp
#pragma once

#include "kg_device.hpp"

namespace kg {

constexpr int kMaxBuckets = 1024;
#ifndef KG_PROBE_N
#define KG_PROBE_N 4
#endif
#ifndef KG_SCATTER_WPE
#define KG_SCATTER_WPE 5
#endif
#ifndef KG_TAG_WPE
#define KG_TAG_WPE 8
#endif
#if KG_SCATTER_WPE
#define KG_SCATTER_REGS __attribute__((amdgpu_waves_per_eu(KG_SCATTER_WPE)))
#else
#define KG_SCATTER_REGS
#endif
#if KG_TAG_WPE
#define KG_TAG_REGS __attribute__((amdgpu_waves_per_eu(KG_TAG_WPE)))
#else
#define KG_TAG_REGS
#endif
#ifndef KG_STAGE_FLUSH
#define KG_STAGE_FLUSH 64
#endif
#ifndef KG_SCATTER_RG
#define KG_SCATTER_RG 6
#endif

#ifndef KG_SCAN_FULL
#define KG_SCAN_FULL 1
#endif

constexpr uint32_t kStageFlush = KG_STAGE_FLUSH;
constexpr int kProbeN = KG_PROBE_N;
#ifndef KG_INDEX_N
#define KG_INDEX_N KG_PROBE_N
#endif
constexpr int kIndexN = KG_INDEX_N;
constexpr uint32_t kUChunk = 512;

constexpr uint64_t kEntInvalid = ~0ull;

template <bool AA>
__device__ __forceinline__ uint32_t window_key(const BlockDesc &bd, uint32_t it, int r, int lane)
{
    const uint32_t ol = (!AA && r >= 3) ? 63u - (uint32_t)lane : (uint32_t)lane;
    return (row_index<AA>(bd, it, r) << 6) | ol;
}
#ifndef KG_SCATTER_WAVES
#define KG_SCATTER_WAVES 16
#endif
constexpr int kScatterWaves = KG_SCATTER_WAVES;
constexpr uint32_t kGroup = 16;

template <bool AA>
inline size_t scatter_lds_bytes(uint32_t n_buckets)
{
    size_t enc = (sizeof(typename WaveLds<AA>::type) + 15) & ~(size_t)15;
    size_t tab = (sizeof(typename WaveLds<AA>::tables) + 15) & ~(size_t)15;
    return enc * kScatterWaves + tab + (size_t)n_buckets * (kGroup * 8 + 8);
}
template <bool AA>
constexpr uint32_t scatter_flush_list_max()
{
    constexpr size_t idle = AA ? sizeof(WaveLdsAa) : KG_SCATTER_RG == 6 ? sizeof(WaveLdsDna) : sizeof(WaveLdsDna::bc);
    return idle / 4 < 64 ? (uint32_t)(idle / 4) : 64u;
}

#ifndef KG_SCATTER_NT
#define KG_SCATTER_NT 1
#endif
__device__ __forceinline__ void store_entry_pair(uint64_t *dst, const ulonglong2 &v)
{
#if KG_SCATTER_NT
    typedef uint64_t u64x2 __attribute__((ext_vector_type(2)));
    u64x2 x; x.x = v.x; x.y = v.y;
    __builtin_nontemporal_store(x, reinterpret_cast<u64x2 *>(dst));
#else
    *reinterpret_cast<ulonglong2 *>(dst) = v;
#endif
}

struct ScatterCold {
    uint32_t *ovf_cursor;
    uint32_t *ovf_bucket;
    uint64_t *ovf_ent;
    uint32_t *lowc_cursor;
    uint32_t *lowc_blocks;
    unsigned long long *ctr;
    Progress *prog;
    uint32_t ovf_cap, pad;
};
static_assert(sizeof(ScatterCold) == 64, "ScatterCold is one 64-byte line");

constexpr unsigned long long kDstOvf = 1ull << 62, kDstNone = ~0ull, kDstDropped = ~0ull - 1;

__device__ __forceinline__ unsigned long long overflow_reserve(const ScatterCold *__restrict__ cold, unsigned long long movf, bool to_ovf,
                                                               uint32_t b, unsigned long long dst)
{
    const int lane = threadIdx.x & 63;
    uint32_t og = 0;
    if (lane == 0) og = atomicAdd(cold->ovf_cursor, (uint32_t)__popcll(movf));
    og = (uint32_t)__builtin_amdgcn_readfirstlane((int)og);
    if (to_ovf) {
        const uint32_t g = og + (uint32_t)__popcll(movf & ((1ull << lane) - 1ull));
        if (g < cold->ovf_cap) { cold->ovf_bucket[g] = b; dst = kDstOvf | ((uint64_t)g * kGroup); }
        else dst = kDstDropped;
    }
    return dst;
}
__device__ __attribute__((noinline, cold)) unsigned long long scatter_overflow_groups(const ScatterCold *__restrict__ cold,
                                                                                     unsigned long long movf, bool to_ovf, uint32_t b,
                                                                                     unsigned long long dst)
{
    return overflow_reserve(cold, movf, to_ovf, b, dst);
}
__device__ __attribute__((noinline, cold)) void scatter_overflow_octets(const ScatterCold *__restrict__ cold, bool full, uint32_t b,
                                                                        uint64_t lo, uint64_t hi)
{
    const int lane = threadIdx.x & 63;
    const bool lead = full && (lane & 7) == 0;
    unsigned long long dst = overflow_reserve(cold, __ballot(lead), lead, b, kDstNone);
    dst = __shfl(dst, lane & ~7);
    if (full && dst != kDstDropped) {
        ulonglong2 v; v.x = lo; v.y = hi;
        store_entry_pair(cold->ovf_ent + (dst & ~kDstOvf) + 2 * ((uint32_t)lane & 7u), v);
    }
}
__device__ __attribute__((noinline, cold)) void scatter_store_overflow(const ScatterCold *__restrict__ cold, unsigned long long to,
                                                                       uint32_t sub, uint64_t lo, uint64_t hi)
{
    ulonglong2 v; v.x = lo; v.y = hi;
    store_entry_pair(cold->ovf_ent + (to & ~kDstOvf) + 2 * sub, v);
}
__device__ __attribute__((noinline, cold)) void scatter_set_aside(const ScatterCold *__restrict__ cold, uint32_t block)
{
    if ((threadIdx.x & 63) == 0) cold->lowc_blocks[atomicAdd(cold->lowc_cursor, 1u)] = block;
}
__device__ __attribute__((noinline, cold)) void scatter_protocol_failure(const ScatterCold *__restrict__ cold)
{
    if ((threadIdx.x & 63) == 0) atomicOr(cold->ovf_cursor + 2, 1u);
}
__device__ __attribute__((noinline, cold)) void scatter_note_beyond(const ScatterCold *__restrict__ cold, uint32_t slot)
{
    progress_note_beyond(cold->prog, slot);
}

struct BlockRows { uint32_t len, j, nk, ibase; };
__device__ __forceinline__ BlockRows rows_of(const BlockDesc &bd) { return BlockRows{bd.len, bd.j, bd.nk, bd.ibase}; }
__device__ __forceinline__ BlockDesc desc_of(const BlockRows &r)
{
    BlockDesc bd;
    bd.soff = 0; bd.len = r.len; bd.j = r.j; bd.nk = r.nk; bd.ibase = r.ibase; bd.seq = 0; bd.pad = 0;
    return bd;
}

template <bool AA, bool SHORT = false, bool PROG = false>
__global__ __launch_bounds__(kWave *kScatterWaves) KG_SCATTER_REGS void part_scatter_kernel(
    const uint8_t *__restrict__ seq, const BlockDesc *__restrict__ blocks, uint32_t block_lo, uint32_t n_blocks ,
    uint32_t limit32 , uint32_t num_sigs , uint32_t m35, uint32_t shift,
    uint32_t n_buckets, uint32_t cap, uint64_t *__restrict__ ent, uint32_t *__restrict__ fill, const ScatterCold *__restrict__ cold,
    uint32_t insert_prio , uint32_t flush_list )
{
    static_assert(SHORT || !PROG, "PROG implies SHORT");
    constexpr int ROWS = AA ? 1 : 6;
    typedef typename WaveLds<AA>::type Enc;
    constexpr size_t enc_bytes = (sizeof(Enc) + 15) & ~(size_t)15;
    extern __shared__ __attribute__((aligned(16))) unsigned char part_lds[];
    const int lane = threadIdx.x & 63, wave = __builtin_amdgcn_readfirstlane((int)(threadIdx.x >> 6));
    Enc &l = *reinterpret_cast<Enc *>(part_lds + enc_bytes * wave);
    typedef typename WaveLds<AA>::tables Tables;
    constexpr size_t tab_bytes = (sizeof(Tables) + 15) & ~(size_t)15;
    Tables &enc_tables = *reinterpret_cast<Tables *>(part_lds + enc_bytes * kScatterWaves);
    uint64_t *buf = reinterpret_cast<uint64_t *>(part_lds + enc_bytes * kScatterWaves + tab_bytes);
    uint32_t *cnt = reinterpret_cast<uint32_t *>(buf + (size_t)n_buckets * kGroup);
    uint32_t *written = cnt + n_buckets;
    uint32_t *flist = reinterpret_cast<uint32_t *>(&l);
    const uint32_t w = blockIdx.x, n_wg = gridDim.x;
    const uint32_t gcap = cap >> 4;
    const uint32_t list_cap = max(min(flush_list, scatter_flush_list_max<AA>()), 1u);
    for (uint32_t b = threadIdx.x; b < n_buckets; b += blockDim.x) { cnt[b] = 0; written[b] = 0; }
    encode_init<AA>(enc_tables, threadIdx.x, blockDim.x);
    __syncthreads();

    uint32_t n_valid = 0;
    bool ran_off = false;
    const uint32_t n_iter = (n_blocks + n_wg * kScatterWaves - 1) / (n_wg * kScatterWaves);
    BlockRows rows_next = {0, 0, 0, 0};
    uint32_t raw_next[4] = {0, 0, 0, 0};
    {
        const uint32_t it0 = w * kScatterWaves + (uint32_t)wave;
        if (it0 < n_blocks) {
            const BlockDesc bd0 = blocks[block_lo + it0];
            load_block_chars<AA>(seq, bd0, lane, raw_next);
            rows_next = rows_of(bd0);
        }
    }
    constexpr int RG = AA ? 1 : KG_SCATTER_RG;
    static_assert(ROWS % RG == 0, "KG_SCATTER_RG must divide 6");
    for (uint32_t iter = 0; iter < n_iter; iter++) {
        const uint32_t it = (iter * n_wg + w) * kScatterWaves + (uint32_t)wave;
        const BlockDesc bd = desc_of(rows_next);
        const bool have = it < n_blocks;
        if (have) {
            uint32_t raw[4] = {raw_next[0], raw_next[1], raw_next[2], raw_next[3]};
            const uint32_t itn = it + n_wg * kScatterWaves;
            if (itn < n_blocks) {
                const BlockDesc bdn = blocks[block_lo + itn];
                load_block_chars<AA>(seq, bdn, lane, raw_next);
                rows_next = rows_of(bdn);
            }
            encode_chars<AA>(l, enc_tables, raw, lane);
        }
        bool lowc = false;
#pragma unroll
        for (int g0 = 0; g0 < ROWS; g0 += RG) {
        uint64_t e[RG];
        uint32_t bk[RG];
        uint32_t pend = 0, nv = 0;
        if (have && !lowc) {
#pragma unroll
            for (int k = 0; k < RG; k++) {
                const int r = g0 + k;
                uint32_t hi, lo, q;
                bool valid = row_halves<AA>(l, r, lane, bd, &hi, &lo);
                const uint32_t slot = split_fast(hi, lo, num_sigs, m35, &q);
                if (valid) nv++;
                if constexpr (SHORT) {
                    if (valid && slot >= limit32) {
                        ran_off = true;
                        if constexpr (PROG) scatter_note_beyond(cold, slot);
                    }
                    valid = valid && slot < limit32;
                }
                bk[k] = slot >> shift;
                const uint32_t low = (q << shift) | (slot & ((1u << shift) - 1u));
                const uint32_t id = window_key<AA>(bd, block_lo + it, r, lane);
                e[k] = ((uint64_t)id << 32) | low;
                if (valid) pend |= 1u << k;
            }
            if (g0 + RG == ROWS) wave_sync();
            if (g0 == 0) {
                const unsigned long long m0 = __ballot((pend & 1u) != 0);
                if (__popcll(m0) >= 32) {
                    const uint32_t lead0 = (uint32_t)__builtin_amdgcn_readlane((int)bk[0], __builtin_ctzll(m0));
                    if (__builtin_expect(__popcll(__ballot((pend & 1u) && bk[0] == lead0)) >= 24, 0)) {
                        scatter_set_aside(cold, block_lo + it);
                        nv = 0;
                        pend = 0;
                        lowc = true;
                        if (RG != ROWS) wave_sync();
                    }
                }
            }
        }
        n_valid += nv;
        uint32_t spins = 0;
        if (insert_prio) set_wave_prio(insert_prio);
        for (;;) {
            uint32_t at[RG], old[RG];
#pragma unroll
            for (int r = 0; r < RG; r++)
                at[r] = (pend & (1u << r)) ? atomicAdd(&cnt[bk[r]], 1u) : kGroup;
#pragma unroll
            for (int r = 0; r < RG; r++) {
                old[r] = 0;
                if (at[r] < kGroup) {
                    buf[(size_t)bk[r] * kGroup + at[r]] = e[r];
                    __builtin_amdgcn_fence(__ATOMIC_RELEASE, "wavefront");
                    old[r] = atomicAdd(&written[bk[r]], 1u);
                }
            }
            __builtin_amdgcn_fence(__ATOMIC_ACQUIRE, "wavefront");
#pragma unroll
            for (int r = 0; r < RG; r++) pend &= ~((uint32_t)(at[r] < kGroup) << r);
            uint32_t at_max = at[0];
#pragma unroll
            for (int r = 1; r < RG; r++) at_max = max(at_max, at[r]);
            uint32_t left = 0;
            auto list_rows = [&](auto again) -> uint32_t {
                uint32_t n = 0;
#pragma unroll
                for (int r = 0; r < RG; r++) {
                    const bool own = decltype(again)::value ? ((left >> r) & 1u) != 0 : (old[r] & 15u) == 15u;
                    const unsigned long long m = __ballot(own);
                    if (m) {
                        const uint32_t rank = __builtin_amdgcn_mbcnt_hi((uint32_t)(m >> 32), __builtin_amdgcn_mbcnt_lo((uint32_t)m, n));
                        if (own && rank < list_cap) {
                            const uint32_t g = decltype(again)::value ? (written[bk[r]] >> 4) - 1u : old[r] >> 4;
                            flist[rank] = (min(g, gcap) << 10) | bk[r];
                            if (decltype(again)::value) left &= ~(1u << r);
                        }
                        n += (uint32_t)__popcll(m);
                    }
                }
                return n;
            };
            uint32_t n_own = list_rows(std::false_type{});
            if (__builtin_expect(n_own > list_cap, 0)) {
                uint32_t k = 0;
#pragma unroll
                for (int r = 0; r < RG; r++) {
                    const bool own = (old[r] & 15u) == 15u;
                    const unsigned long long m = __ballot(own);
                    const uint32_t rank = __builtin_amdgcn_mbcnt_hi((uint32_t)(m >> 32), __builtin_amdgcn_mbcnt_lo((uint32_t)m, k));
                    if (own && rank >= list_cap) left |= 1u << r;
                    k += (uint32_t)__popcll(m);
                }
            }
            while (n_own) {
                const uint32_t n_list = min(n_own, list_cap);
                wave_sync();
                for (uint32_t p0 = 0; p0 < n_list; p0 += 8) {
                    const uint32_t want = p0 + ((uint32_t)lane >> 3), sub = (uint32_t)lane & 7u;
                    if (want < n_list) {
                        const uint32_t d = flist[want];
                        const uint32_t fb = d & (uint32_t)(kMaxBuckets - 1), g = d >> 10;
                        const ulonglong2 v = *reinterpret_cast<const ulonglong2 *>(buf + (size_t)fb * kGroup + 2 * sub);
                        __builtin_amdgcn_fence(__ATOMIC_RELEASE, "wavefront");
                        if (sub == 0) cnt[fb] = 0;
                        const bool full = g >= gcap;
                        if (!full) {
                            unsigned char *to = reinterpret_cast<unsigned char *>(ent) + (mul24_wide(__umul24(fb, n_wg) + w, cap) << 3);
                            store_entry_pair(reinterpret_cast<uint64_t *>(to + ((g << 7) | (sub << 4))), v);
                        }
                        if (__builtin_expect(__ballot(full) != 0, 0)) scatter_overflow_octets(cold, full, fb, v.x, v.y);
                    }
                }
                wave_sync();
                if (__builtin_expect(n_own <= list_cap, 1)) break;
                n_own = list_rows(std::true_type{});
            }
            if (!__ballot(pend != 0)) break;
            {
                const int rp = pend ? __builtin_ctz(pend) : 0;
                uint32_t pb = bk[0];
#pragma unroll
                for (int r = 1; r < RG; r++)
                    if (rp == r) pb = bk[r];
                for (uint32_t polls = 0; polls < 64; polls++) {
                    if (__ballot(pend != 0 && __hip_atomic_load(&cnt[pb], __ATOMIC_RELAXED, __HIP_MEMORY_SCOPE_WORKGROUP) < kGroup)) break;
                    __builtin_amdgcn_s_sleep(2);
                }
            }
            if (__builtin_expect(++spins > (1u << 20) || __ballot(at_max >= (1u << 28)), 0)) {
                scatter_protocol_failure(cold);
                break;
            }
        }
        if (insert_prio) set_wave_prio(0);
        }
    }
    __syncthreads();
    const uint32_t per_wave = (n_buckets + kScatterWaves - 1) / kScatterWaves;
    const uint32_t b_end = min((uint32_t)(wave + 1) * per_wave, n_buckets);
    for (uint32_t b0 = (uint32_t)wave * per_wave; b0 < b_end; b0 += 64) {
        const uint32_t b = b0 + (uint32_t)lane;
        const uint32_t wr = b < b_end ? written[b] : 0u;
        const uint32_t c = wr & 15u, g = wr >> 4;
        unsigned long long dst = kDstNone;
        bool to_ovf = false;
        if (c > 0) {
            for (uint32_t k = c; k < kGroup; k++) buf[(size_t)b * kGroup + k] = kEntInvalid;
            if (g < gcap) dst = ((uint64_t)b * n_wg + w) * cap + ((uint64_t)g << 4);
            else to_ovf = true;
        }
        const unsigned long long movf = __ballot(to_ovf);
        if (movf) dst = scatter_overflow_groups(cold, movf, to_ovf, b, dst);
        unsigned long long m = __ballot(dst != kDstNone);
        wave_sync();
        while (m) {
            int src_lane = -1;
            unsigned long long mm = m;
#pragma unroll
            for (int o = 0; o < 8; o++) {
                const int ln = mm ? __builtin_ctzll(mm) : -1;
                if (mm) mm &= mm - 1;
                if ((lane >> 3) == o) src_lane = ln;
            }
            m = mm;
            const int sl = src_lane < 0 ? 0 : src_lane;
            const uint32_t fb = (uint32_t)__shfl((int)b, sl);
            const unsigned long long to = __shfl(dst, sl);
            if (src_lane >= 0) {
                const uint32_t sub = (uint32_t)lane & 7u;
                const ulonglong2 v = *reinterpret_cast<const ulonglong2 *>(buf + (size_t)fb * kGroup + 2 * sub);
                if (__builtin_expect((to & kDstOvf) != 0, 0)) {
                    if (to != kDstDropped) scatter_store_overflow(cold, to, sub, v.x, v.y);
                } else {
                    store_entry_pair(ent + to + 2 * sub, v);
                }
            }
        }
    }
    for (uint32_t b = threadIdx.x; b < n_buckets; b += blockDim.x)
        fill[(uint64_t)b * n_wg + w] = min((written[b] + 15u) >> 4, gcap) << 4;
    for (int off = 32; off > 0; off >>= 1) n_valid += __shfl_down(n_valid, off);
    unsigned long long *ctr = cold->ctr;
    if (lane == 0 && n_valid) atomicAdd(&ctr[0], (unsigned long long)n_valid);
    if constexpr (SHORT) flush_ran_off(ran_off, ctr, lane);
}

constexpr int kLowcWaves = 4;
template <bool AA>
__global__ __launch_bounds__(64 * kLowcWaves) void lowc_blocks_kernel(
    const uint8_t *__restrict__ seq, const BlockDesc *__restrict__ blocks, const uint32_t *__restrict__ lowc_cursor,
    const uint32_t *__restrict__ lowc_blocks, uint64_t limit, uint32_t num_sigs, uint32_t m35, uint32_t shift, uint32_t n_regions,
    uint32_t cap, uint64_t *__restrict__ ent, uint32_t *__restrict__ fill, uint32_t *ovf_cursor, uint32_t ovf_cap,
    uint32_t *__restrict__ ovf_bucket, uint64_t *__restrict__ ovf_ent, unsigned long long *ctr, Progress *prog)
{
    constexpr int ROWS = AA ? 1 : 6;
    __shared__ typename WaveLds<AA>::type lds[kLowcWaves];
    __shared__ typename WaveLds<AA>::tables enc_tables;
    const int lane = threadIdx.x & 63, wave = threadIdx.x >> 6;
    typename WaveLds<AA>::type &l = lds[wave];
    const uint32_t n_list = *lowc_cursor;
    if (n_list == 0) return;
    encode_init<AA>(enc_tables, threadIdx.x, blockDim.x);
    __syncthreads();
    const uint32_t limit32 = limit < 0xFFFFFFFFull ? (uint32_t)limit : 0xFFFFFFFFu;
    unsigned long long n_valid = 0;
    bool ran_off = false;
    uint32_t pool_at = 0, pool_end = 0;
    auto pool_flush = [&]() {
        for (uint32_t g = pool_at + ((uint32_t)lane >> 4); g < pool_end && g < ovf_cap; g += 4) {
            if ((lane & 15) == 0) ovf_bucket[g] = 0;
            ovf_ent[(uint64_t)g * kGroup + ((uint32_t)lane & 15u)] = kEntInvalid;
        }
        pool_at = pool_end;
    };
    auto ovf_groups = [&](uint32_t lead, uint32_t ng) -> uint64_t * {
        if (pool_end - pool_at < ng) {
            pool_flush();
            const uint32_t want = ng > 32u ? ng : 32u;
            uint32_t g0 = 0;
            if (lane == 0) g0 = atomicAdd(ovf_cursor, want);
            g0 = (uint32_t)__builtin_amdgcn_readfirstlane((int)g0);
            pool_at = g0; pool_end = g0 + want;
        }
        const uint32_t g = pool_at;
        pool_at += ng;
        if (g + ng > ovf_cap) return nullptr;
        if ((uint32_t)lane < ng) ovf_bucket[g + lane] = lead;
        return ovf_ent + (uint64_t)g * kGroup;
    };
    for (uint32_t i = blockIdx.x * kLowcWaves + (uint32_t)wave; i < n_list; i += gridDim.x * kLowcWaves) {
        const uint32_t it = (uint32_t)__builtin_amdgcn_readfirstlane((int)lowc_blocks[i]);
        const BlockDesc bd = blocks[it];
        encode_block<AA>(l, enc_tables, seq, bd, lane);
        const uint32_t region_w = it % n_regions;
        for (int r = 0; r < ROWS; r++) {
            uint32_t hi, lo, q;
            bool valid = row_halves<AA>(l, r, lane, bd, &hi, &lo);
            const uint32_t slot = split_fast(hi, lo, num_sigs, m35, &q);
            if (valid) n_valid++;
            if (valid && slot >= limit32) { ran_off = true; if (prog) progress_note_beyond(prog, slot); }
            bool pend = valid && slot < limit32;
            const uint32_t bkt = slot >> shift;
            const uint64_t e = ((uint64_t)window_key<AA>(bd, it, r, lane) << 32) | ((q << shift) | (slot & ((1u << shift) - 1u)));
            for (int pass = 0; pass < 4; pass++) {
                const unsigned long long mp = __ballot(pend);
                if (__popcll(mp) < 16) break;
                const uint32_t lead = (uint32_t)__builtin_amdgcn_readlane((int)bkt, __builtin_ctzll(mp));
                const bool mine = pend && bkt == lead;
                const unsigned long long same = __ballot(mine);
                const uint32_t n = (uint32_t)__popcll(same);
                if (n < 8) break;
                const uint32_t rank = (uint32_t)__popcll(same & ((1ull << lane) - 1ull));
                const uint64_t region = (uint64_t)lead * n_regions + region_w;
                uint32_t rel = cap;
                if (lane == 0 && *const_cast<volatile uint32_t *>(&fill[region]) < cap) rel = atomicAdd(&fill[region], n);
                rel = (uint32_t)__builtin_amdgcn_readfirstlane((int)rel);
                if (rel + n <= cap) {
                    if (mine) ent[region * cap + rel + rank] = e;
                } else {
                    if (rel < cap && (uint32_t)lane < cap - rel) ent[region * cap + rel + lane] = kEntInvalid;
                    const uint32_t npad = (n + kGroup - 1) & ~(kGroup - 1);
                    uint64_t *dst = ovf_groups(lead, npad / kGroup);
                    if (dst) {
                        if (mine) dst[rank] = e;
                        if ((uint32_t)lane < npad - n) dst[n + lane] = kEntInvalid;
                    }
                }
                if (mine) pend = false;
            }
            if (pend) {
                const uint64_t region = (uint64_t)bkt * n_regions + region_w;
                const uint32_t rel = atomicAdd(&fill[region], 1u);
                if (rel < cap) { ent[region * cap + rel] = e; pend = false; }
            }
            for (;;) {
                const unsigned long long mp = __ballot(pend);
                if (!mp) break;
                const uint32_t lead = (uint32_t)__builtin_amdgcn_readlane((int)bkt, __builtin_ctzll(mp));
                const bool mine = pend && bkt == lead;
                const unsigned long long same = __ballot(mine);
                const uint32_t n = (uint32_t)__popcll(same);
                const uint32_t npad = (n + kGroup - 1) & ~(kGroup - 1);
                const uint32_t rank = (uint32_t)__popcll(same & ((1ull << lane) - 1ull));
                uint64_t *dst = ovf_groups(lead, npad / kGroup);
                if (dst) {
                    if (mine) dst[rank] = e;
                    if ((uint32_t)lane < npad - n) dst[n + lane] = kEntInvalid;
                }
                if (mine) pend = false;
            }
        }
        wave_sync();
    }
    pool_flush();
    for (int off = 32; off > 0; off >>= 1) n_valid += __shfl_down(n_valid, off);
    if (lane == 0 && n_valid) atomicAdd(&ctr[0], n_valid);
    flush_ran_off(ran_off, ctr, lane);
}

struct UListState { unsigned long long base; uint32_t used; bool have; };

template <bool AA, int N, bool COUNTERS>
__device__ __forceinline__ void probe_entries(const TableView &tab, uint32_t b, uint32_t shift, const uint64_t (&e)[N],
                                              kg_hit *__restrict__ ulist, uint32_t *__restrict__ chunk_used,
                                              unsigned long long *cursor, uint64_t ulist_cap, UListState &u,
                                              unsigned long long &ctr_slots, bool &ran_off, int lane, Progress *prog)
{
    uint64_t val[N], slot[N];
    bool valid[N];
    uint32_t id[N], fp[N];
#pragma unroll
    for (int k = 0; k < N; k++) {
        valid[k] = e[k] != kEntInvalid;
        const uint32_t low = (uint32_t)e[k];
        id[k] = (uint32_t)(e[k] >> 32);
        slot[k] = ((uint64_t)b << shift) | (low & ((1u << shift) - 1u));
        val[k] = (uint64_t)(low >> shift) * tab.num_sigs + slot[k];
        fp[k] = tag_qs(low >> shift, slot[k]);
    }
    Payload pay[N];
    unsigned long long ctr_dummy = 0;
    uint32_t fslot[N];
#pragma unroll
    for (int k = 0; k < N; k++) fslot[k] = 0;
    const uint32_t foundm = probe_n<N, COUNTERS>(tab, val, slot, fp, valid, pay, ctr_dummy, ctr_slots, ran_off, COUNTERS ? prog : nullptr,
                                                 COUNTERS ? fslot : nullptr);
    uint32_t cnt[N], rank[N], total = 0;
#pragma unroll
    for (int k = 0; k < N; k++) {
        const bool f = (foundm >> k) & 1u;
        const unsigned long long m = __ballot(f);
        cnt[k] = (uint32_t)__popcll(m);
        rank[k] = (uint32_t)__popcll(m & ((1ull << lane) - 1ull));
        total += cnt[k];
    }
    if (total) {
        if (u.used + total > kUChunk) {
            if (lane == 0 && u.have && u.base + kUChunk <= ulist_cap) chunk_used[u.base / kUChunk] = u.used;
            unsigned long long nb = 0;
            if (lane == 0) nb = atomicAdd(cursor, (unsigned long long)kUChunk);
            nb = ((unsigned long long)__builtin_amdgcn_readfirstlane((uint32_t)(nb >> 32)) << 32) |
                 (unsigned long long)__builtin_amdgcn_readfirstlane((uint32_t)nb);
            u.base = nb; u.used = 0; u.have = true;
        }
        if (u.base + kUChunk <= ulist_cap) {
            uint32_t at = u.used;
#pragma unroll
            for (int k = 0; k < N; k++) {
                if ((foundm >> k) & 1u) {
                    kg_hit h;
                    h.container = id[k];
                    h.from0InProt = (int32_t)fslot[k];
                    h.oI = pay[k].oI; h.avgOffFromEnd = pay[k].avg; h.fI = pay[k].fI; h.functionWt = pay[k].wt;
                    ulist[u.base + at + rank[k]] = h;
                }
                at += cnt[k];
            }
        }
        u.used += total;
    }
}

struct CandRec { uint32_t home, quo, id, walked; };
constexpr uint32_t kWalkOn = 0x80000000u;
constexpr uint32_t kScanOn = 0x40000000u;
constexpr uint32_t kWalkedMask = 0x3FFFFFFFu;
static_assert(sizeof(CandRec) == 16, "CandRec must be 16 bytes");

__device__ __forceinline__ unsigned long long chunk_reserve(UListState &u, uint32_t total, uint32_t *__restrict__ chunk_used,
                                                            unsigned long long *cursor, uint64_t cap, int lane)
{
    if (u.used + total > kUChunk) {
        if (lane == 0 && u.have && u.base + kUChunk <= cap) chunk_used[u.base / kUChunk] = u.used;
        unsigned long long nb = 0;
        if (lane == 0) nb = atomicAdd(cursor, (unsigned long long)kUChunk);
        nb = ((unsigned long long)__builtin_amdgcn_readfirstlane((uint32_t)(nb >> 32)) << 32) |
             (unsigned long long)__builtin_amdgcn_readfirstlane((uint32_t)nb);
        u.base = nb; u.used = 0; u.have = true;
    }
    const unsigned long long at = u.base + u.used;
    u.used += total;
    return u.base + kUChunk <= cap ? at : ~0ull;
}

__device__ __forceinline__ void chunk_finish(const UListState &u, uint32_t *__restrict__ chunk_used, uint64_t cap, int lane)
{
    if (lane == 0 && u.have && u.base + kUChunk <= cap) chunk_used[u.base / kUChunk] = u.used;
}

template <bool COUNTERS>
__global__ __launch_bounds__(256) KG_TAG_REGS void bucket_tag_kernel(
    const uint8_t *__restrict__ tags, uint64_t limit, uint64_t num_sigs, const uint64_t *__restrict__ ent,
    const uint32_t *__restrict__ fill, uint32_t n_regions, uint32_t cap, uint32_t n_buckets, uint32_t shift,
    uint32_t grab ,
    uint32_t *next_region ,
    CandRec *__restrict__ cand, uint32_t *__restrict__ cand_used, unsigned long long *cand_cursor, uint64_t cand_cap,
    unsigned long long *ctr, Progress *prog )
{
    constexpr int N = kProbeN;
    const uint32_t lim32 = (uint32_t)limit;
    __shared__ uint32_t s_region;
    __shared__ __attribute__((aligned(16))) CandRec s_stage[4][kStageFlush + 64];
    CandRec *stage = s_stage[__builtin_amdgcn_readfirstlane((int)(threadIdx.x >> 6))];
    uint32_t sfill = 0;
    const int lane = threadIdx.x & 63;
    unsigned long long ctr_slots = 0;
    bool ran_off = false;
    UListState u;
    u.base = 0; u.used = kUChunk; u.have = false;

    const uint32_t kGrab = grab;
    const uint32_t grabs_per_region = (cap + kGrab - 1) / kGrab;
    const uint32_t n_grabs = n_regions * grabs_per_region;
    const uint32_t xg = blockIdx.x & 7u;
    const uint32_t n_tickets = xg < n_buckets ? ((n_buckets - xg + 7u) / 8u) * n_grabs : 0u;
    for (;;) {
        __syncthreads();
        if (threadIdx.x == 0) s_region = atomicAdd(&next_region[xg * 32u], 1u);
        __syncthreads();
        const uint32_t tk = s_region;
        if (tk >= n_tickets) break;
        const uint32_t b = xg + 8u * (tk / n_grabs), g = tk % n_grabs;
        const uint32_t w = g / grabs_per_region, g0 = (g % grabs_per_region) * kGrab;
        const uint32_t fraw = fill[(uint64_t)b * n_regions + w];
        uint32_t n = cap;
        const uint64_t *src = ent + ((uint64_t)b * n_regions + w) * cap;
        for (uint32_t c0 = g0; c0 < n && c0 < g0 + kGrab; c0 += 256u * N) {
            const uint32_t bound = n;
            uint32_t low[N], id[N], fp[N], skip[N], walked[N];
            uint32_t vmask = 0;
            Tags16 tg[N];
            const uint32_t smask = (1u << shift) - 1u, bbase = b << shift;
            uint64_t ev[N];
#pragma unroll
            for (int k = 0; k < N; k++) {
                const uint32_t i = c0 + (uint32_t)k * 256u + threadIdx.x;
                ev[k] = i < bound ? __builtin_nontemporal_load(src + i) : kEntInvalid;
            }
            if (c0 == g0) {
                uint32_t f = fraw;
                asm volatile("; fill first used here" : "+s"(f));
                n = min(f, cap);
            }
#pragma unroll
            for (int k = 0; k < N; k++) {
                const uint64_t e = c0 + (uint32_t)k * 256u + threadIdx.x < n ? ev[k] : kEntInvalid;
                if (e != kEntInvalid) vmask |= 1u << k;
                low[k] = (uint32_t)e;
                id[k] = (uint32_t)(e >> 32);
                const uint32_t home = bbase | (low[k] & smask);
                fp[k] = tag_qs(low[k] >> shift, home);
                const uint32_t cur = (uint32_t)probe_window(home, &skip[k]);
                if ((vmask >> k) & 1u) tg[k] = load_tags(tags + cur);
            }
            uint32_t candm = 0, walkm = 0;
#pragma unroll
            for (int k = 0; k < N; k++) {
                walked[k] = 0;
                if ((vmask >> k) & 1u) {
                    bool emp;
                    const int i = first_stop(tg[k], fp[k], &emp, skip[k]);
                    walked[k] = (uint32_t)i - skip[k];
                    if (i == 16) { candm |= 1u << k; walkm |= 1u << k; }
                    else if (!emp) candm |= 1u << k;
                    else {
                        const uint32_t home = bbase | (low[k] & smask), at = home + walked[k];
                        if (at >= lim32) ran_off = true;
                        if (COUNTERS) {
                            ctr_slots += (at < lim32 ? at + 1u : lim32) - home;
                            if (prog) progress_note_walk(prog, home, at, lim32);
                        }
                    }
                }
            }
#pragma unroll
            for (int k = 0; k < N; k++) {
                const unsigned long long m = __ballot((candm >> k) & 1u);
                if (!m) continue;
                if ((candm >> k) & 1u) {
                    CandRec c;
                    c.home = bbase | (low[k] & smask); c.quo = low[k] >> shift;
                    c.id = id[k]; c.walked = walked[k] | (((walkm >> k) & 1u) ? kWalkOn : 0u);
                    stage[sfill + (uint32_t)__popcll(m & ((1ull << lane) - 1ull))] = c;
                }
                sfill += (uint32_t)__popcll(m);
                while (sfill >= kStageFlush) {
                    wave_sync();
                    const unsigned long long at = chunk_reserve(u, kStageFlush, cand_used, cand_cursor, cand_cap, lane);
                    if ((uint32_t)lane < kStageFlush) {
                        const ulonglong2 out = *reinterpret_cast<const ulonglong2 *>(stage + lane);
                        if (at != ~0ull) stream_store16(cand + at + (uint32_t)lane, &out);
                    }
                    sfill -= kStageFlush;
                    wave_sync();
                    if ((uint32_t)lane < sfill) {
                        const ulonglong2 rest = *reinterpret_cast<const ulonglong2 *>(stage + kStageFlush + lane);
                        *reinterpret_cast<ulonglong2 *>(stage + lane) = rest;
                    }
                    wave_sync();
                }
            }
        }
    }
    if (sfill) {
        wave_sync();
        const CandRec out = stage[(uint32_t)lane < sfill ? lane : 0];
        const unsigned long long at = chunk_reserve(u, sfill, cand_used, cand_cursor, cand_cap, lane);
        if (at != ~0ull && (uint32_t)lane < sfill) stream_store16(cand + at + (uint32_t)lane, &out);
    }
    chunk_finish(u, cand_used, cand_cap, lane);
    flush_ran_off(ran_off, ctr, lane);
    if (COUNTERS) {
        for (int off = 32; off > 0; off >>= 1) ctr_slots += __shfl_down(ctr_slots, off);
        if (lane == 0) atomicAdd(&ctr[1], ctr_slots);
    }
}

template <int N, int R, bool EXACT, bool PROG = false>
__global__ __launch_bounds__(256) KG_TAG_REGS void bucket_index_kernel(
    const uint8_t *__restrict__ bidx, uint32_t tail_start,
    const uint64_t *__restrict__ ent, const uint32_t *__restrict__ fill, uint32_t n_regions , uint32_t cap, uint32_t n_buckets,
    uint32_t shift, uint32_t grab ,
    uint32_t *next_region ,
    CandRec *__restrict__ cand, uint32_t *__restrict__ cand_used, unsigned long long *cand_cursor, uint64_t cand_cap,
    unsigned long long *ctr, uint32_t prio , Progress *prog )
{
    static_assert(N % R == 0, "R must divide N");
    constexpr int PER = N / R;
    __shared__ uint32_t s_region;
    __shared__ uint32_t s_lut[256];
    __shared__ __attribute__((aligned(16))) CandRec s_stage[4][kStageFlush + 64];
    CandRec *stage = s_stage[__builtin_amdgcn_readfirstlane((int)(threadIdx.x >> 6))];
    uint32_t sfill = 0;
    const int lane = threadIdx.x & 63;
    bool ran_off = false;
    UListState u;
    u.base = 0; u.used = kUChunk; u.have = false;
    s_lut[threadIdx.x] = bidx_decode(threadIdx.x);
    if (prio) set_wave_prio(prio);

    const uint32_t kGrab = grab;
    const uint32_t grabs_per_region = (cap + kGrab - 1) / kGrab;
    const uint32_t n_grabs = (n_regions / R) * grabs_per_region;
    const uint32_t xg = blockIdx.x & 7u;
    const uint32_t n_tickets = xg < n_buckets ? ((n_buckets - xg + 7u) / 8u) * n_grabs : 0u;
    constexpr uint32_t all_walk = EXACT ? 0u : kBidxInexact;
    for (;;) {
        __syncthreads();
        if (threadIdx.x == 0) s_region = atomicAdd(&next_region[xg * 32u], 1u);
        __syncthreads();
        const uint32_t tk = s_region;
        if (tk >= n_tickets) break;
        const uint32_t b = xg + 8u * (tk / n_grabs), g = tk % n_grabs;
        const uint32_t w = (g / grabs_per_region) * R, g0 = (g % grabs_per_region) * kGrab;
        uint32_t fraw[R], n[R], nmax = cap;
#pragma unroll
        for (int r = 0; r < R; r++) { fraw[r] = fill[(uint64_t)b * n_regions + w + r]; n[r] = cap; }
        const uint64_t *src = ent + ((uint64_t)b * n_regions + w) * cap;
        const uint32_t smask = (1u << shift) - 1u, bbase = b << shift;
        uint32_t d_lo = 0, d_hi = 0, pmin = ~0u, pmax1 = 0;
        if (PROG) {
            const uint64_t s0 = (uint64_t)b << shift, s1 = (((uint64_t)b + 1) << shift) - 1;
#pragma unroll
            for (int k = 1; k <= 10; k++) { d_lo += prog->lo[k] <= s0 ? 1u : 0u; d_hi += prog->lo[k] <= s1 ? 1u : 0u; }
        }
        for (uint32_t c0 = g0; c0 < nmax && c0 < g0 + kGrab; c0 += 256u * PER) {
            uint64_t ev[N];
#pragma unroll
            for (int k = 0; k < N; k++) {
                const int r = k / PER;
                const uint32_t i = c0 + (uint32_t)(k % PER) * 256u + threadIdx.x;
                ev[k] = i < n[r] ? __builtin_nontemporal_load(src + (uint64_t)r * cap + i) : kEntInvalid;
            }
            if (c0 == g0) {
                nmax = 0;
#pragma unroll
                for (int r = 0; r < R; r++) {
                    uint32_t f = fraw[r];
                    asm volatile("; fill first used here" : "+s"(f));
                    n[r] = min(f, cap);
                    nmax = max(nmax, n[r]);
                }
            }
            uint32_t code[N], vmask = 0;
#pragma unroll
            for (int k = 0; k < N; k++) {
                if (c0 + (uint32_t)(k % PER) * 256u + threadIdx.x >= n[k / PER]) ev[k] = kEntInvalid;
                code[k] = 0;
                if (ev[k] != kEntInvalid) {
                    vmask |= 1u << k;
                    code[k] = bidx[bbase | ((uint32_t)ev[k] & smask)];
                }
            }
            uint32_t candm = 0, walkm = 0, wd[N];
#pragma unroll
            for (int k = 0; k < N; k++) wd[k] = s_lut[code[k]];
#pragma unroll
            for (int k = 0; k < N; k++) {
                const uint32_t q = (uint32_t)ev[k] >> shift;
                const uint32_t c = EXACT ? q : q % kBidxClasses;
                const uint32_t listed = (wd[k] >> c) & 1u;
                candm |= listed << k;
                walkm |= (listed & ((wd[k] | all_walk) >> 31)) << k;
                ran_off = ran_off || (((vmask >> k) & 1u) && !listed && (bbase | ((uint32_t)ev[k] & smask)) >= tail_start);
            }
            if (PROG) {
                if (d_lo == d_hi) {
#pragma unroll
                    for (int k = 0; k < N; k++) {
                        const uint32_t h = bbase | ((uint32_t)ev[k] & smask);
                        if ((vmask >> k) & 1u) pmin = min(pmin, h);
                        if (((vmask & ~candm) >> k) & 1u) pmax1 = max(pmax1, h + 1u);
                    }
                } else {
                    for (int k = 0; k < N; k++)
                        if ((vmask >> k) & 1u) progress_note_home(prog, d_lo, d_hi, bbase | ((uint32_t)ev[k] & smask), (candm >> k) & 1u);
                }
            }
#pragma unroll
            for (int k = 0; k < N; k++) {
                const unsigned long long m = __ballot((candm >> k) & 1u);
                if (!m) continue;
                if ((candm >> k) & 1u) {
                    CandRec c;
                    c.home = bbase | ((uint32_t)ev[k] & smask); c.quo = (uint32_t)ev[k] >> shift;
                    c.id = (uint32_t)(ev[k] >> 32); c.walked = ((walkm >> k) & 1u) ? kWalkOn : kScanOn;
                    stage[sfill + (uint32_t)__popcll(m & ((1ull << lane) - 1ull))] = c;
                }
                sfill += (uint32_t)__popcll(m);
                while (sfill >= kStageFlush) {
                    wave_sync();
                    const unsigned long long at = chunk_reserve(u, kStageFlush, cand_used, cand_cursor, cand_cap, lane);
                    if ((uint32_t)lane < kStageFlush) {
                        const ulonglong2 out = *reinterpret_cast<const ulonglong2 *>(stage + lane);
                        if (at != ~0ull) stream_store16(cand + at + (uint32_t)lane, &out);
                    }
                    sfill -= kStageFlush;
                    wave_sync();
                    if ((uint32_t)lane < sfill) {
                        const ulonglong2 rest = *reinterpret_cast<const ulonglong2 *>(stage + kStageFlush + lane);
                        *reinterpret_cast<ulonglong2 *>(stage + lane) = rest;
                    }
                    wave_sync();
                }
            }
        }
        if (PROG && d_lo == d_hi) progress_note_homes(prog, d_lo, pmin, pmax1);
    }
    if (sfill) {
        wave_sync();
        const CandRec out = stage[(uint32_t)lane < sfill ? lane : 0];
        const unsigned long long at = chunk_reserve(u, sfill, cand_used, cand_cursor, cand_cap, lane);
        if (at != ~0ull && (uint32_t)lane < sfill) stream_store16(cand + at + (uint32_t)lane, &out);
    }
    chunk_finish(u, cand_used, cand_cap, lane);
    flush_ran_off(ran_off, ctr, lane);
}

template <bool AA, bool COUNTERS, bool PROG = false>
__global__ __launch_bounds__(256) void verify_kernel(
    const uint8_t *__restrict__ entries, const uint8_t *__restrict__ tags, uint64_t limit, uint64_t num_sigs, uint64_t magic,
    const CandRec *__restrict__ cand, const uint32_t *__restrict__ cand_used, const unsigned long long *cand_cursor,
    uint64_t cand_cap, kg_hit *__restrict__ ulist, uint32_t *__restrict__ chunk_used, unsigned long long *cursor,
    uint64_t ulist_cap, unsigned long long *ctr, Progress *prog ,
    uint32_t prio )
{
    const int lane = threadIdx.x & 63;
    const uint32_t wave_global = __builtin_amdgcn_readfirstlane(blockIdx.x * 4 + (threadIdx.x >> 6));
    const uint32_t n_waves = gridDim.x * 4;
    if (prio) set_wave_prio(prio);
    TableView tab;
    tab.entries = entries; tab.tags = tags; tab.limit = limit; tab.num_sigs = num_sigs; tab.magic = magic; tab.m35 = 0;
    const unsigned long long cur = *cand_cursor;
    const uint32_t n_chunks = (uint32_t)((cur < cand_cap ? cur : cand_cap) / kUChunk);
    unsigned long long ctr_slots = 0;
    bool ran_off = false;
    UListState u;
    u.base = 0; u.used = kUChunk; u.have = false;
    for (uint32_t c = wave_global; c < n_chunks; c += n_waves) {
        const uint32_t used = cand_used[c];
        for (uint32_t k0 = 0; k0 < used; k0 += 64) {
            const bool act = k0 + (uint32_t)lane < used;
            CandRec r;
            r.home = 0; r.quo = 0; r.id = 0; r.walked = 0;
            if (act) {
                const kg_u32x4 cv = __builtin_nontemporal_load(reinterpret_cast<const kg_u32x4 *>(cand + (uint64_t)c * kUChunk + k0 + lane));
                r.home = cv.x; r.quo = cv.y; r.id = cv.z; r.walked = cv.w;
            }
            const uint64_t quo = r.quo, home = r.home;
            const uint64_t val = quo * num_sigs + home;
            uint64_t s = home + (r.walked & kWalkedMask);
            bool found = false;
            Entry e;
            e.key = 0; e.oI = e.avg = e.fI = 0; e.wt = 0.f;
            if (act && (r.walked & kScanOn)) {
#if KG_SCAN_FULL
                if (s < limit) {
                    const uint64_t s1 = s + 1 < limit ? s + 1 : s, s2 = s + 2 < limit ? s + 2 : s;
                    const Entry e0 = load_entry(tab, s);
                    const uint2 k1 = *reinterpret_cast<const uint2 *>(tab.entries + s1 * 24);
                    const uint2 k2 = *reinterpret_cast<const uint2 *>(tab.entries + s2 * 24);
                    const uint32_t vlo = (uint32_t)val, vhi = (uint32_t)(val >> 32);
                    if (e0.key == (int64_t)val) { found = true; e = e0; }
                    else if (s + 1 < limit && k1.x == vlo && k1.y == vhi) { found = true; s += 1; e = load_entry(tab, s); }
                    else if (s + 2 < limit && k2.x == vlo && k2.y == vhi) { found = true; s += 2; e = load_entry(tab, s); }
                    else s += 3;
                }
#endif
                while (!found) {
                    if (s >= limit) { s = limit; ran_off = true; break; }
                    const uint64_t s1 = s + 1 < limit ? s + 1 : s, s2 = s + 2 < limit ? s + 2 : s;
                    const uint2 k0 = *reinterpret_cast<const uint2 *>(tab.entries + s * 24);
                    const uint2 k1 = *reinterpret_cast<const uint2 *>(tab.entries + s1 * 24);
                    const uint2 k2 = *reinterpret_cast<const uint2 *>(tab.entries + s2 * 24);
                    const uint32_t vlo = (uint32_t)val, vhi = (uint32_t)(val >> 32);
                    if (k0.x == vlo && k0.y == vhi) found = true;
                    else if (s + 1 < limit && k1.x == vlo && k1.y == vhi) { found = true; s += 1; }
                    else if (s + 2 < limit && k2.x == vlo && k2.y == vhi) { found = true; s += 2; }
                    if (found) { e = load_entry(tab, s); break; }
                    s += 3;
                }
                if (COUNTERS) {
                    ctr_slots += (s < limit ? s + 1 : limit) - home;
                    if (prog) progress_note_walk(prog, home, s, limit);
                } else if (PROG) {
                    progress_note_walk(prog, home, s, limit);
                }
            } else if (act) {
                if (!(r.walked & kWalkOn)) {
                    e = load_entry(tab, s);
                    found = e.key == (int64_t)val;
                    if (!found) s += 1;
                }
                if (!found) {
                    const uint32_t f = tag_qs(quo, home);
                    for (;;) {
                        if (s >= limit) { s = limit; ran_off = true; break; }
                        const Tags16 x = load_tags(tab.tags + s);
                        bool emp;
                        const int i = first_stop(x, f, &emp);
                        if (i == 16) { s += 16; continue; }
                        s += (uint64_t)i;
                        if (emp) { if (s >= limit) ran_off = true; break; }
                        e = load_entry(tab, s);
                        if (e.key == (int64_t)val) { found = true; break; }
                        s += 1;
                    }
                }
                if (COUNTERS) {
                    ctr_slots += (s < limit ? s + 1 : limit) - home;
                    if (prog) progress_note_walk(prog, home, s, limit);
                } else if (PROG) {
                    progress_note_walk(prog, home, s, limit);
                }
            }
            const unsigned long long m = __ballot(found);
            const uint32_t total = (uint32_t)__popcll(m);
            if (total) {
                const unsigned long long at = chunk_reserve(u, total, chunk_used, cursor, ulist_cap, lane);
                if (at != ~0ull && found) {
                    kg_hit h;
                    h.container = r.id;
                    h.from0InProt = (int32_t)(uint32_t)s;
                    h.oI = e.oI; h.avgOffFromEnd = e.avg; h.fI = e.fI; h.functionWt = e.wt;
                    stream_store_hit(ulist + at + (uint32_t)__popcll(m & ((1ull << lane) - 1ull)), h);
                }
            }
        }
    }
    chunk_finish(u, chunk_used, ulist_cap, lane);
    flush_ran_off(ran_off, ctr, lane);
    if (COUNTERS) {
        for (int off = 32; off > 0; off >>= 1) ctr_slots += __shfl_down(ctr_slots, off);
        if (lane == 0) atomicAdd(&ctr[1], ctr_slots);
    }
}

template <bool AA, bool COUNTERS, bool PROG = false>
__global__ __launch_bounds__(256) void overflow_probe_kernel(
    const uint8_t *__restrict__ entries, const uint8_t *__restrict__ tags, uint64_t limit, uint64_t num_sigs, uint64_t magic,
    const uint32_t *__restrict__ ovf_bucket, const uint64_t *__restrict__ ovf_ent, const uint32_t *__restrict__ ovf_cursor,
    uint32_t ovf_cap, uint32_t shift, kg_hit *__restrict__ ulist, uint32_t *__restrict__ chunk_used, unsigned long long *cursor, uint64_t ulist_cap,
    unsigned long long *ctr, Progress *prog)
{
    const int lane = threadIdx.x & 63;
    const uint32_t wave_global = __builtin_amdgcn_readfirstlane(blockIdx.x * 4 + (threadIdx.x >> 6));
    const uint32_t n_waves = gridDim.x * 4;
    TableView tab;
    tab.entries = entries; tab.tags = tags; tab.limit = limit; tab.num_sigs = num_sigs; tab.magic = magic; tab.m35 = 0;
    unsigned long long ctr_slots = 0;
    bool ran_off = false;
    UListState u;
    u.base = 0; u.used = kUChunk; u.have = false;
    const uint32_t n_groups = min(*ovf_cursor, ovf_cap);
    for (uint32_t g = wave_global; g < n_groups; g += n_waves) {
        const uint32_t b = ovf_bucket[g];
        uint64_t e[1];
        e[0] = lane < (int)kGroup ? ovf_ent[(uint64_t)g * kGroup + lane] : kEntInvalid;
        probe_entries<AA, 1, COUNTERS || PROG>(tab, b, shift, e, ulist, chunk_used, cursor, ulist_cap, u, ctr_slots, ran_off, lane, prog);
    }
    if (lane == 0 && u.have && u.base + kUChunk <= ulist_cap) chunk_used[u.base / kUChunk] = u.used;
    flush_ran_off(ran_off, ctr, lane);
    if (COUNTERS) {
        for (int off = 32; off > 0; off >>= 1) ctr_slots += __shfl_down(ctr_slots, off);
        if (lane == 0) atomicAdd(&ctr[1], ctr_slots);
    }
}

__global__ void chunk_base_kernel(const uint64_t *chunk_total, uint64_t *base, uint64_t *grand_total)
{
    const uint64_t b = base[0] + *chunk_total;
    base[1] = b;
    if (grand_total) *grand_total = b;
}

}
```

Baseline: 132.6 billion residues/s.

## Fuse hit histogram into verify/probe and first partition pass, drop hist kernel

```diff
diff --git a/kmergutsjava_amd/csrc/kg_host.hpp b/kmergutsjava_amd/csrc/kg_host.hpp
--- a/kmergutsjava_amd/csrc/kg_host.hpp
+++ b/kmergutsjava_amd/csrc/kg_host.hpp
@@ -220,7 +220,6 @@
     kg::ScatterCold h_cold[kMaxChunks] = {};
     kg::CallsCold *d_calls_cold = nullptr;
     kg::CallsCold h_calls_cold = {};
-    size_t hist_lds = 48 * 1024;
     size_t place_lds[2] = {48 * 1024, 48 * 1024};
     hipEvent_t ev[kEvCount] = {};
     uint64_t *h_pin = nullptr;
diff --git a/kmergutsjava_amd/csrc/kg_host_plan.hpp b/kmergutsjava_amd/csrc/kg_host_plan.hpp
--- a/kmergutsjava_amd/csrc/kg_host_plan.hpp
+++ b/kmergutsjava_amd/csrc/kg_host_plan.hpp
@@ -141,6 +141,7 @@
     pl.cap = (uint32_t)cap64;
     pl.n_regions = (uint64_t)pl.buckets * n_wg;
     pl.ovf_cap = env_u32("KG_PART_OVF_GROUPS", (uint32_t)std::min<uint64_t>(1u << 23, std::max<uint64_t>(65536, pl.n_regions * pl.cap / 16 / 8)));
+    pl.gshift = env_knob("KG_ORDER_GSHIFT", 10u, 6u, 12u);
     while (pl.gshift < 12 && ((max_chunk * PER) >> pl.gshift) + 2 > 8192) pl.gshift++;
     pl.groups_stride = (uint32_t)(((max_chunk * PER) >> pl.gshift) + 2);
     if (pl.groups_stride > kg::kMaxGroups) return fail(KG_ERR_LIMIT, "a chunk of the batch holds more than 2^26 window rows");
diff --git a/kmergutsjava_amd/csrc/kg_host_scan.hpp b/kmergutsjava_amd/csrc/kg_host_scan.hpp
--- a/kmergutsjava_amd/csrc/kg_host_scan.hpp
+++ b/kmergutsjava_amd/csrc/kg_host_scan.hpp
@@ -135,7 +135,7 @@
     uint32_t *d_lowc = nullptr;
     kg::RowGeo *d_geo = nullptr;
     uint64_t *d_pc = nullptr;
-    uint32_t *d_ghist = nullptr, *d_gbase = nullptr, *d_gcur1 = nullptr, *d_gcur2 = nullptr, *d_gtile = nullptr;
+    uint32_t *d_d1hist = nullptr, *d_ghist = nullptr, *d_gbase = nullptr, *d_gcur1 = nullptr, *d_gcur2 = nullptr, *d_gtile = nullptr;
     uint64_t ucap = 0, ccap = 0;
     size_t cused_stride = 0, candused_stride = 0;
     kg_hit *d_ulist = nullptr, *d_sortA = nullptr, *d_sortB = nullptr;
@@ -152,8 +152,18 @@
     kg::CandRec *cand;
     unsigned long long *ucur, *ccur;
     uint64_t *base, *ctot;
-    uint32_t *ghist, *gbase, *gcur1, *gcur2, *gtile;
+    uint32_t *d1hist, *ghist, *gbase, *gcur1, *gcur2, *gtile;
 };
+
+struct ChunkGroups { uint64_t row_lo, row_hi; uint32_t g0, n_groups; };
+ChunkGroups chunk_groups(const PartPlan &pl, const ChunkView &v, uint32_t per)
+{
+    ChunkGroups g;
+    g.row_lo = (uint64_t)v.lo * per; g.row_hi = g.row_lo + (uint64_t)v.nb * per;
+    g.g0 = (uint32_t)(g.row_lo >> pl.gshift);
+    g.n_groups = v.nb ? (uint32_t)(((g.row_hi - 1) >> pl.gshift) - g.g0 + 1) : 1u;
+    return g;
+}
 
 ChunkView chunk_view(const PartPlan &pl, const PartBuffers &pb, uint32_t c)
 {
@@ -169,6 +179,7 @@
     v.cand = pb.d_cand + (uint64_t)c * pb.ccap;
     v.ucur = (unsigned long long *)(pb.d_pc + kPcUcur + c); v.ccur = (unsigned long long *)(pb.d_pc + kPcCcur + c);
     v.base = pb.d_pc + kPcBase + c; v.ctot = pb.d_pc + kPcCtot + c;
+    v.d1hist = pb.d_d1hist + (size_t)c * kg::kHDigits;
     v.ghist = pb.d_ghist + (size_t)c * pl.groups_stride; v.gbase = pb.d_gbase + (size_t)c * (pl.groups_stride + 1);
     v.gcur1 = pb.d_gcur1 + (size_t)c * (kg::kHDigits + 1); v.gcur2 = pb.d_gcur2 + (size_t)c * pl.groups_stride;
     v.gtile = pb.d_gtile + (size_t)c * (kg::kHDigits + 1);
@@ -216,6 +227,8 @@
     const hipStream_t s2 = t->stream2, s3 = t->stream3;
     uint32_t *lowc_cursor = v.ovfc + kOvfLowc, *lowc = pb.d_lowc + v.lo;
     const uint32_t limit32 = (uint32_t)std::min<uint64_t>(t->limit, 0xFFFFFFFFull);
+    const ChunkGroups cg = chunk_groups(pl, v, AA ? 1 : 6);
+    const kg::D1Count dc{cg.g0, 6u + pl.gshift, cg.n_groups, v.d1hist};
     scatter_variant(scatter_variant_of(cx), [&](auto is_short, auto prog) {
         constexpr bool SHORT = decltype(is_short)::value, PROG = decltype(prog)::value;
         hipLaunchKernelGGL((kg::part_scatter_kernel<AA, SHORT, PROG>), dim3(pl.n_wg), dim3(kg::kWave * kg::kScatterWaves), pl.scatter_lds,
@@ -254,10 +267,10 @@
         constexpr bool COUNTERS = decltype(walks)::value == 1, PROG = decltype(walks)::value == 2;
         hipLaunchKernelGGL((kg::verify_kernel<AA, COUNTERS, PROG>), dim3(pl.verify_grid), dim3(256), 0, s3, t->d_entries, t->d_tags, t->limit,
                            (uint64_t)t->num_sigs, t->magic, v.cand, v.candused, v.ccur, pb.ccap, v.ulist, v.cused, v.ucur, pb.ucap, d_ctr,
-                           d_prog, pl.verify_prio);
+                           d_prog, pl.verify_prio, dc);
         hipLaunchKernelGGL((kg::overflow_probe_kernel<AA, COUNTERS, PROG>), dim3(pl.ovf_grid), dim3(256), 0, s3, t->d_entries, t->d_tags,
                            t->limit, (uint64_t)t->num_sigs, t->magic, v.ovf_bucket, v.ovf_ent, v.ovfc, pl.ovf_cap, pl.shift, v.ulist,
-                           v.cused, v.ucur, pb.ucap, d_ctr, d_prog);
+                           v.cused, v.ucur, pb.ucap, d_ctr, d_prog, dc);
     });
     HIP_TRY(hipEventRecord(t->pev[kPevVerified + v.c], s3));
     HIP_TRY(hipGetLastError());
@@ -278,12 +291,10 @@
         HIP_TRY(hipStreamWaitEvent(s, t->ev[kEvScattered], 0));
     }
     HIP_TRY(hipStreamWaitEvent(s, t->pev[kPevVerified + c], 0));
-    const uint64_t row_lo = (uint64_t)v.lo * PER, row_hi = row_lo + (uint64_t)v.nb * PER;
-    const uint32_t g0 = (uint32_t)(row_lo >> gshift);
-    const uint32_t n_groups = v.nb ? (uint32_t)(((row_hi - 1) >> gshift) - g0 + 1) : 1u;
-    hipLaunchKernelGGL(kg::hit_hist_kernel, dim3(pl.order_grid), dim3(kg::kHThreads), (size_t)n_groups * 4, s, v.ulist, v.cused, v.ucur, pb.ucap,
-                       g0, 6u + gshift, n_groups, v.ghist);
-    hipLaunchKernelGGL(kg::group_scan_kernel, dim3(1), dim3(kg::kGsThreads), 0, s, v.ghist, n_groups, v.gbase, v.gcur1, v.gcur2, v.ctot, v.gtile);
+    const ChunkGroups cg = chunk_groups(pl, v, PER);
+    const uint64_t row_lo = cg.row_lo, row_hi = cg.row_hi;
+    const uint32_t g0 = cg.g0, n_groups = cg.n_groups;
+    hipLaunchKernelGGL(kg::d1_scan_kernel, dim3(1), dim3(kg::kHDigits), 0, s, v.d1hist, n_groups, v.gcur1, v.ctot);
     if (pl.n_os && c) HIP_TRY(hipStreamWaitEvent(s, t->pev[kPevBase + c - 1], 0));
     hipLaunchKernelGGL(kg::chunk_base_kernel, dim3(1), dim3(1), 0, s, v.ctot, v.base, last ? cx.d_totals : (uint64_t *)nullptr);
     if (pl.n_os) HIP_TRY(hipEventRecord(t->pev[kPevBase + c], s));
@@ -293,9 +304,10 @@
         HIP_TRY(hipEventRecord(t->pev[kPevTotals], s));
     }
     hipLaunchKernelGGL((kg::hit_partition_kernel<true>), dim3(pl.order_grid), dim3(kg::kHThreads), 0, s, v.ulist, v.cused, v.ucur, pb.ucap,
-                       v.gbase, n_groups, g0, 6u + gshift, v.gcur1, v.sortA, pb.ucap, v.gtile);
+                       v.gbase, n_groups, g0, 6u + gshift, v.gcur1, v.sortA, pb.ucap, v.gtile, v.ghist);
+    hipLaunchKernelGGL(kg::group_scan_kernel, dim3(1), dim3(kg::kGsThreads), 0, s, v.ghist, n_groups, v.gbase, v.gcur2, v.gtile);
     hipLaunchKernelGGL((kg::hit_partition_kernel<false>), dim3(pl.order_grid), dim3(kg::kHThreads), 0, s, v.sortA, v.cused, v.ucur, pb.ucap,
-                       v.gbase, n_groups, g0, 6u + gshift, v.gcur2, v.sortB, pb.ucap, v.gtile);
+                       v.gbase, n_groups, g0, 6u + gshift, v.gcur2, v.sortB, pb.ucap, v.gtile, (uint32_t *)nullptr);
     hipLaunchKernelGGL((kg::group_place_kernel<AA>), dim3(std::min(n_groups, 256u * 8u)), dim3(kg::kHThreads),
                        kg::group_place_lds(gshift, pl.place_staged), s,
                        v.sortB, v.gbase, n_groups, g0, gshift, (uint32_t)row_lo, (uint32_t)row_hi, pb.d_geo, (uint64_t)cx.b.n_rows,
@@ -319,6 +331,7 @@
     if ((rc = sc.get(&pb.d_ovfc, kOvfWords * kMaxChunks))) return rc;
     if ((rc = sc.get(&pb.d_lowc, (size_t)cx.b.nblocks + 1))) return rc;
     if ((rc = sc.get(&pb.d_geo, (size_t)cx.b.n_rows))) return rc;
+    if ((rc = sc.get(&pb.d_d1hist, (size_t)kg::kHDigits * n_chunks))) return rc;
     if ((rc = sc.get(&pb.d_ghist, (size_t)groups_stride * n_chunks))) return rc;
     if ((rc = sc.get(&pb.d_gbase, (size_t)(groups_stride + 1) * n_chunks))) return rc;
     if ((rc = sc.get(&pb.d_gcur1, (size_t)(kg::kHDigits + 1) * n_chunks))) return rc;
@@ -328,10 +341,6 @@
         const size_t want_lds = kg::group_place_lds(pl.gshift, pl.gshift == 10);
         HIP_TRY(hipFuncSetAttribute((const void *)kg::group_place_kernel<AA>, hipFuncAttributeMaxDynamicSharedMemorySize, (int)want_lds));
         t->place_lds[AA ? 1 : 0] = want_lds;
-    }
-    if (groups_stride * 4u > t->hist_lds) {
-        HIP_TRY(hipFuncSetAttribute((const void *)kg::hit_hist_kernel, hipFuncAttributeMaxDynamicSharedMemorySize, (int)(groups_stride * 4u)));
-        t->hist_lds = groups_stride * 4u;
     }
     if ((rc = sc.get(&pb.d_pc, kPcWords))) return rc;
     const int sv = scatter_variant_of(cx);
@@ -382,6 +391,7 @@
                                {cx.d_totals, kTotWords * 2},
                                {pb.d_ovfc, kOvfWords * kMaxChunks},
                                {pb.d_next, (uint64_t)pl.next_stride * n_chunks},
+                               {pb.d_d1hist, (uint64_t)kg::kHDigits * n_chunks},
                                {pb.d_ghist, (uint64_t)pl.groups_stride * n_chunks}})))
             return rc;
         if ((rc = upload_scatter_cold(cx, pl, pb))) return rc;
diff --git a/kmergutsjava_amd/csrc/kg_order.hpp b/kmergutsjava_amd/csrc/kg_order.hpp
--- a/kmergutsjava_amd/csrc/kg_order.hpp
+++ b/kmergutsjava_amd/csrc/kg_order.hpp
@@ -8,7 +8,6 @@
 constexpr uint32_t kHThreads = 512;
 constexpr uint32_t kHPer = 4;
 constexpr uint32_t kHTile = kHThreads * kHPer;
-constexpr uint32_t kHDigits = 128;
 constexpr uint32_t kMaxGroups = kHDigits * kHDigits;
 
 struct RowGeo { uint32_t container; int32_t pos_first; };
@@ -28,35 +27,35 @@
     geo[row_index<AA>(bd, it, (int)r)] = g;
 }
 
-__global__ __launch_bounds__(kHThreads) void hit_hist_kernel(const kg_hit *__restrict__ ulist, const uint32_t *__restrict__ chunk_used,
-                                                             const unsigned long long *__restrict__ cursor, uint64_t ulist_cap,
-                                                             uint32_t g0, uint32_t gs , uint32_t n_groups,
-                                                             uint32_t *ghist )
-{
-    extern __shared__ uint32_t h_lds[];
-    for (uint32_t g = threadIdx.x; g < n_groups; g += kHThreads) h_lds[g] = 0;
-    __syncthreads();
-    const unsigned long long cur = *cursor;
-    const uint32_t n_chunks = (uint32_t)((cur < ulist_cap ? cur : ulist_cap) / kUChunk);
-    for (uint32_t c = blockIdx.x; c < n_chunks; c += gridDim.x) {
-        const uint32_t used = chunk_used[c];
-        for (uint32_t k = threadIdx.x; k < used; k += kHThreads) {
-            const uint32_t g = (ulist[(uint64_t)c * kUChunk + k].container >> gs) - g0;
-            if (g < n_groups) atomicAdd(&h_lds[g], 1u);
-        }
-    }
-    __syncthreads();
-    for (uint32_t g = threadIdx.x; g < n_groups; g += kHThreads)
-        if (h_lds[g]) atomicAdd(&ghist[g], h_lds[g]);
+__global__ __launch_bounds__(kHDigits) void d1_scan_kernel(const uint32_t *__restrict__ d1hist, uint32_t n_groups, uint32_t *__restrict__ cur1,
+                                                           uint64_t *total_out)
+{
+    __shared__ uint32_t first_half;
+    const uint32_t d = threadIdx.x, lane = d & 63u;
+    const uint32_t n_d1 = (n_groups + kHDigits - 1) / kHDigits;
+    const uint32_t c = d < n_d1 ? d1hist[d] : 0u;
+    uint32_t incl = c;
+    for (int off = 1; off < 64; off <<= 1) {
+        const uint32_t y = __shfl_up(incl, off);
+        if ((int)lane >= off) incl += y;
+    }
+    if (d == 63) first_half = incl;
+    __syncthreads();
+    const uint32_t before = d >= 64 ? first_half : 0u;
+    if (d < n_d1) cur1[d] = before + incl - c;
+    if (d == kHDigits - 1) {
+        cur1[n_d1] = before + incl;
+        *total_out = before + incl;
+    }
 }
 
 constexpr uint32_t kGsThreads = 256, kGsPer = 4;
 __global__ __launch_bounds__(kGsThreads) void group_scan_kernel(const uint32_t *__restrict__ ghist, uint32_t n_groups, uint32_t *__restrict__ gbase,
-                                                                uint32_t *__restrict__ cur1, uint32_t *__restrict__ cur2, uint64_t *total_out,
-                                                                uint32_t *__restrict__ tile_start)
+                                                                uint32_t *__restrict__ cur2, uint32_t *__restrict__ tile_start)
 {
     __shared__ uint32_t wsum[kGsThreads / 64];
     __shared__ uint32_t carry;
+    __shared__ uint32_t d1s[kHDigits + 1];
     if (threadIdx.x == 0) carry = 0;
     __syncthreads();
     const int lane = threadIdx.x & 63, wave = threadIdx.x >> 6;
@@ -89,7 +88,7 @@
             if (i < n_groups) {
                 gbase[i] = e;
                 cur2[i] = e;
-                if ((i & (kHDigits - 1)) == 0) cur1[i / kHDigits] = e;
+                if ((i & (kHDigits - 1)) == 0) d1s[i / kHDigits] = e;
             }
             e += x[k];
         }
@@ -100,12 +99,11 @@
     const uint32_t n_d1 = (n_groups + kHDigits - 1) / kHDigits;
     if (threadIdx.x == 0) {
         gbase[n_groups] = carry;
-        cur1[n_d1] = carry;
-        *total_out = carry;
+        d1s[n_d1] = carry;
     }
     __syncthreads();
     const uint32_t d = threadIdx.x;
-    const uint32_t t = d < n_d1 ? (cur1[d + 1] - cur1[d] + kHTile - 1) / kHTile : 0u;
+    const uint32_t t = d < n_d1 ? (d1s[d + 1] - d1s[d] + kHTile - 1) / kHTile : 0u;
     uint32_t incl = t;
     for (int off = 1; off < 64; off <<= 1) {
         const uint32_t y = __shfl_up(incl, off);
@@ -119,31 +117,51 @@
         if (d == kHDigits - 1) tile_start[kHDigits] = before + incl;
     }
 }
+
+constexpr uint32_t kHFirstStage = kHTile / 2;
+constexpr uint32_t kGhLds = 8448;
+constexpr uint32_t kGhFlushTiles = 65535u / kHTile;
+static_assert(kGhFlushTiles * kHTile <= 65535u && kGhFlushTiles >= 1, "a 16-bit group counter could wrap between two flushes");
+static_assert(kHTile % kUChunk == 0 && kGhLds % 2 == 0, "tiles of whole reservation chunks; two counters to a word");
 
 template <bool FIRST>
 __global__ __launch_bounds__(kHThreads) void hit_partition_kernel(const kg_hit *__restrict__ in, const uint32_t *__restrict__ chunk_used,
                                                                   const unsigned long long *__restrict__ cursor, uint64_t in_cap,
                                                                   const uint32_t *__restrict__ gbase, uint32_t n_groups, uint32_t g0, uint32_t gs,
                                                                   uint32_t *cur, kg_hit *__restrict__ out, uint64_t out_cap,
-                                                                  const uint32_t *__restrict__ tile_start)
-{
-    __shared__ __attribute__((aligned(16))) kg_hit stage[kHTile];
+                                                                  const uint32_t *__restrict__ tile_start,
+                                                                  uint32_t *ghist )
+{
+    constexpr uint32_t PER = kHPer, TILE = kHTile, STAGE = FIRST ? kHFirstStage : kHTile;
+    __shared__ __attribute__((aligned(16))) kg_hit stage[STAGE];
     __shared__ uint32_t hist[kHDigits], cnt[kHDigits], sbase[kHDigits], gb[kHDigits];
+    __shared__ uint32_t ghl[FIRST ? kGhLds / 2 : 1];
     const uint32_t tid = threadIdx.x, lane = tid & 63u, wave = tid >> 6;
     if (tid < kHDigits) hist[tid] = 0;
     const uint32_t n_d1 = (n_groups + kHDigits - 1) / kHDigits;
+    const uint32_t gh_words = (min(n_groups, kGhLds) + 1u) / 2u;
     uint32_t n_res = 0;
     if (FIRST) {
         const unsigned long long cc = *cursor;
         n_res = (uint32_t)((cc < in_cap ? cc : in_cap) / kUChunk);
-    }
+        for (uint32_t w = tid; w < gh_words; w += kHThreads) ghl[w] = 0;
+    }
+    auto flush_groups = [&]() {
+        for (uint32_t w = tid; w < gh_words; w += kHThreads) {
+            const uint32_t x = ghl[w];
+            if (x) {
+                if (x & 0xFFFFu) atomicAdd(&ghist[2u * w], x & 0xFFFFu);
+                if (x >> 16) atomicAdd(&ghist[2u * w + 1u], x >> 16);
+                ghl[w] = 0;
+            }
+        }
+    };
     __shared__ uint32_t tstart[kHDigits + 1];
-    if (!FIRST) {
-        if (tid <= kHDigits) tstart[tid] = tile_start[tid];
-        __syncthreads();
-    }
-    const uint32_t n_items = FIRST ? (n_res + kHTile / kUChunk - 1) / (kHTile / kUChunk) : tstart[kHDigits];
+    if (!FIRST && tid <= kHDigits) tstart[tid] = tile_start[tid];
+    __syncthreads();
+    const uint32_t n_items = FIRST ? (n_res + TILE / kUChunk - 1) / (TILE / kUChunk) : tstart[kHDigits];
     {
+        uint32_t since_flush = 0;
         for (uint32_t item = blockIdx.x; item < n_items; item += gridDim.x) {
             uint32_t d1 = 0, tile = item;
             if (!FIRST) {
@@ -157,19 +175,19 @@
             }
             const uint32_t seg_lo = FIRST ? 0u : gbase[d1 * kHDigits];
             const uint32_t seg_hi = FIRST ? 0u : gbase[min((d1 + 1) * kHDigits, n_groups)];
-            kg_hit rec[kHPer];
-            uint32_t dr[kHPer];
-#pragma unroll
-            for (uint32_t k = 0; k < kHPer; k++) {
+            kg_hit rec[PER];
+            uint32_t dr[PER];
+#pragma unroll
+            for (uint32_t k = 0; k < PER; k++) {
                 const uint32_t i = k * kHThreads + tid;
                 bool ok;
                 uint64_t at;
                 if (FIRST) {
-                    const uint32_t c = tile * (kHTile / kUChunk) + i / kUChunk;
+                    const uint32_t c = tile * (TILE / kUChunk) + i / kUChunk;
                     ok = c < n_res && (i % kUChunk) < chunk_used[c];
                     at = (uint64_t)c * kUChunk + (i % kUChunk);
                 } else {
-                    at = (uint64_t)seg_lo + (uint64_t)tile * kHTile + i;
+                    at = (uint64_t)seg_lo + (uint64_t)tile * TILE + i;
                     ok = at < seg_hi;
                 }
                 dr[k] = ~0u;
@@ -179,6 +197,10 @@
                     if (g < n_groups) {
                         const uint32_t d = FIRST ? g / kHDigits : g % kHDigits;
                         dr[k] = (d << 16) | atomicAdd(&hist[d], 1u);
+                        if (FIRST) {
+                            if (g < kGhLds) atomicAdd(&ghl[g >> 1], 1u << (16u * (g & 1u)));
+                            else atomicAdd(&ghist[g], 1u);
+                        }
                     }
                 }
             }
@@ -197,26 +219,40 @@
             }
             __syncthreads();
             const uint32_t first_half = sbase[63] + cnt[63];
-#pragma unroll
-            for (uint32_t k = 0; k < kHPer; k++)
-                if (dr[k] != ~0u) {
-                    const uint32_t d = dr[k] >> 16;
-                    stage[sbase[d] + (d >= 64 ? first_half : 0u) + (dr[k] & 0xFFFFu)] = rec[k];
-                }
-            __syncthreads();
-            const uint64_t *stage64 = reinterpret_cast<const uint64_t *>(stage);
-            uint64_t *out64 = reinterpret_cast<uint64_t *>(out);
-            for (uint32_t d = wave; d < kHDigits; d += kHThreads / 64u) {
-                const uint32_t n = cnt[d];
-                if (n == 0) continue;
-                const uint32_t s0 = sbase[d] + (d >= 64 ? first_half : 0u);
-                const uint64_t o0 = gb[d];
-                const uint32_t n_ok = o0 >= out_cap ? 0u : (uint32_t)min((uint64_t)n, out_cap - o0);
-                for (uint32_t i = lane; i < 3u * n_ok; i += 64u) stream_store8(out64 + o0 * 3u + i, stage64[(uint64_t)s0 * 3u + i]);
-            }
-            __syncthreads();
-        }
-    }
+            const uint32_t n_tile = first_half + sbase[kHDigits - 1] + cnt[kHDigits - 1];
+            for (uint32_t r0 = 0; r0 < TILE && r0 < n_tile; r0 += STAGE) {
+#pragma unroll
+                for (uint32_t k = 0; k < PER; k++)
+                    if (dr[k] != ~0u) {
+                        const uint32_t d = dr[k] >> 16;
+                        const uint32_t pos = sbase[d] + (d >= 64 ? first_half : 0u) + (dr[k] & 0xFFFFu);
+                        if (STAGE == TILE || (pos >= r0 && pos - r0 < STAGE)) stage[pos - r0] = rec[k];
+                    }
+                __syncthreads();
+                const uint64_t *stage64 = reinterpret_cast<const uint64_t *>(stage);
+                uint64_t *out64 = reinterpret_cast<uint64_t *>(out);
+                for (uint32_t d = wave; d < kHDigits; d += kHThreads / 64u) {
+                    const uint32_t n = cnt[d];
+                    if (n == 0) continue;
+                    const uint32_t s0 = sbase[d] + (d >= 64 ? first_half : 0u);
+                    const uint64_t o0 = gb[d];
+                    const uint32_t n_ok = o0 >= out_cap ? 0u : (uint32_t)min((uint64_t)n, out_cap - o0);
+                    const uint32_t a = max(s0, r0), b = min(s0 + n_ok, r0 + STAGE);
+                    if (a >= b) continue;
+                    const uint64_t *src = stage64 + (uint64_t)(a - r0) * 3u;
+                    uint64_t *dst = out64 + (o0 + (a - s0)) * 3u;
+                    for (uint32_t i = lane; i < 3u * (b - a); i += 64u) stream_store8(dst + i, src[i]);
+                }
+                __syncthreads();
+            }
+            if (FIRST && ++since_flush == kGhFlushTiles) {
+                flush_groups();
+                since_flush = 0;
+                __syncthreads();
+            }
+        }
+    }
+    if (FIRST) flush_groups();
 }
 
 constexpr uint32_t kPlaceOut = 1536;
diff --git a/kmergutsjava_amd/csrc/kg_partition.hpp b/kmergutsjava_amd/csrc/kg_partition.hpp
--- a/kmergutsjava_amd/csrc/kg_partition.hpp
+++ b/kmergutsjava_amd/csrc/kg_partition.hpp
@@ -42,6 +42,7 @@
 #endif
 constexpr int kIndexN = KG_INDEX_N;
 constexpr uint32_t kUChunk = 512;
+constexpr uint32_t kHDigits = 128;
 
 constexpr uint64_t kEntInvalid = ~0ull;
 
@@ -520,11 +521,33 @@
 
 struct UListState { unsigned long long base; uint32_t used; bool have; };
 
+struct D1Count { uint32_t g0, gs , n_groups; uint32_t *hist ; };
+
+__device__ __forceinline__ void d1_begin(uint32_t *d1_lds)
+{
+    if (threadIdx.x < kHDigits) d1_lds[threadIdx.x] = 0;
+    __syncthreads();
+}
+__device__ __forceinline__ void d1_count(uint32_t *d1_lds, const D1Count &dc, uint32_t key)
+{
+    const uint32_t g = (key >> dc.gs) - dc.g0;
+    if (g < dc.n_groups) atomicAdd(&d1_lds[g / kHDigits], 1u);
+}
+__device__ __forceinline__ void d1_end(const uint32_t *d1_lds, const D1Count &dc)
+{
+    __syncthreads();
+    if (threadIdx.x < kHDigits) {
+        const uint32_t n = d1_lds[threadIdx.x];
+        if (n) atomicAdd(&dc.hist[threadIdx.x], n);
+    }
+}
+
 template <bool AA, int N, bool COUNTERS>
 __device__ __forceinline__ void probe_entries(const TableView &tab, uint32_t b, uint32_t shift, const uint64_t (&e)[N],
                                               kg_hit *__restrict__ ulist, uint32_t *__restrict__ chunk_used,
                                               unsigned long long *cursor, uint64_t ulist_cap, UListState &u,
-                                              unsigned long long &ctr_slots, bool &ran_off, int lane, Progress *prog)
+                                              unsigned long long &ctr_slots, bool &ran_off, int lane, Progress *prog,
+                                              uint32_t *d1_lds, const D1Count &dc)
 {
     uint64_t val[N], slot[N];
     bool valid[N];
@@ -573,6 +596,7 @@
                     h.from0InProt = (int32_t)fslot[k];
                     h.oI = pay[k].oI; h.avgOffFromEnd = pay[k].avg; h.fI = pay[k].fI; h.functionWt = pay[k].wt;
                     ulist[u.base + at + rank[k]] = h;
+                    d1_count(d1_lds, dc, id[k]);
                 }
                 at += cnt[k];
             }
@@ -883,8 +907,10 @@
     const CandRec *__restrict__ cand, const uint32_t *__restrict__ cand_used, const unsigned long long *cand_cursor,
     uint64_t cand_cap, kg_hit *__restrict__ ulist, uint32_t *__restrict__ chunk_used, unsigned long long *cursor,
     uint64_t ulist_cap, unsigned long long *ctr, Progress *prog ,
-    uint32_t prio )
-{
+    uint32_t prio , D1Count dc)
+{
+    __shared__ uint32_t d1_lds[kHDigits];
+    d1_begin(d1_lds);
     const int lane = threadIdx.x & 63;
     const uint32_t wave_global = __builtin_amdgcn_readfirstlane(blockIdx.x * 4 + (threadIdx.x >> 6));
     const uint32_t n_waves = gridDim.x * 4;
@@ -984,6 +1010,7 @@
                     h.from0InProt = (int32_t)(uint32_t)s;
                     h.oI = e.oI; h.avgOffFromEnd = e.avg; h.fI = e.fI; h.functionWt = e.wt;
                     stream_store_hit(ulist + at + (uint32_t)__popcll(m & ((1ull << lane) - 1ull)), h);
+                    d1_count(d1_lds, dc, r.id);
                 }
             }
         }
@@ -994,6 +1021,7 @@
         for (int off = 32; off > 0; off >>= 1) ctr_slots += __shfl_down(ctr_slots, off);
         if (lane == 0) atomicAdd(&ctr[1], ctr_slots);
     }
+    d1_end(d1_lds, dc);
 }
 
 template <bool AA, bool COUNTERS, bool PROG = false>
@@ -1001,8 +1029,10 @@
     const uint8_t *__restrict__ entries, const uint8_t *__restrict__ tags, uint64_t limit, uint64_t num_sigs, uint64_t magic,
     const uint32_t *__restrict__ ovf_bucket, const uint64_t *__restrict__ ovf_ent, const uint32_t *__restrict__ ovf_cursor,
     uint32_t ovf_cap, uint32_t shift, kg_hit *__restrict__ ulist, uint32_t *__restrict__ chunk_used, unsigned long long *cursor, uint64_t ulist_cap,
-    unsigned long long *ctr, Progress *prog)
-{
+    unsigned long long *ctr, Progress *prog, D1Count dc)
+{
+    __shared__ uint32_t d1_lds[kHDigits];
+    d1_begin(d1_lds);
     const int lane = threadIdx.x & 63;
     const uint32_t wave_global = __builtin_amdgcn_readfirstlane(blockIdx.x * 4 + (threadIdx.x >> 6));
     const uint32_t n_waves = gridDim.x * 4;
@@ -1017,7 +1047,7 @@
         const uint32_t b = ovf_bucket[g];
         uint64_t e[1];
         e[0] = lane < (int)kGroup ? ovf_ent[(uint64_t)g * kGroup + lane] : kEntInvalid;
-        probe_entries<AA, 1, COUNTERS || PROG>(tab, b, shift, e, ulist, chunk_used, cursor, ulist_cap, u, ctr_slots, ran_off, lane, prog);
+        probe_entries<AA, 1, COUNTERS || PROG>(tab, b, shift, e, ulist, chunk_used, cursor, ulist_cap, u, ctr_slots, ran_off, lane, prog, d1_lds, dc);
     }
     if (lane == 0 && u.have && u.base + kUChunk <= ulist_cap) chunk_used[u.base / kUChunk] = u.used;
     flush_ran_off(ran_off, ctr, lane);
@@ -1025,6 +1055,7 @@
         for (int off = 32; off > 0; off >>= 1) ctr_slots += __shfl_down(ctr_slots, off);
         if (lane == 0) atomicAdd(&ctr[1], ctr_slots);
     }
+    d1_end(d1_lds, dc);
 }
 
 __global__ void chunk_base_kernel(const uint64_t *chunk_total, uint64_t *base, uint64_t *grand_total)
```

New measurement: 133.1 billion residues/s (median of 6 runs). Within noise of the previous version (+0.4%).
